# thourihan/DeepfakeDetection

Measured on AMD Instinct MI355X. Metric: train images/sec @224^2 (EfficientNet-B0), higher is better.
Workload: dtype bf16; 1 GPU; EfficientNet-b0 (timm flavour) 224x224 train step: bf16 fwd + label-smoothed CE + bwd + AdamW, random-init weights, 2 classes; per_gpu_batch=256, global_batch=256, parallelism=dp1, launch=hipgraph

## Files before the change

### deepfakedetection_amd/_lib.py

```python

from __future__ import annotations

import ctypes
from ctypes import POINTER, Structure, c_double, c_float, c_int, c_int64, c_long, c_size_t, c_uint32, c_void_p
from pathlib import Path

import os as _os

LIB_PATH = Path(_os.environ.get("DFD_LIB_PATH") or Path(__file__).resolve().parent / "libdfd_hip.so")

DFD_OK = 0
ERRORS = {-1: "DFD_EINVAL", -2: "DFD_EUNSUPPORTED", -3: "DFD_ELAUNCH", -4: "DFD_EWORKSPACE"}
F32, BF16 = 0, 1
ACT_NONE, ACT_SILU, ACT_RELU, ACT_GELU = 0, 1, 2, 3
PRO_NONE, PRO_BN_ACT, PRO_BN_ACT_GATE, PRO_AFFINE2 = 0, 1, 2, 3
MAX_PARTIALS = 1024
ADAMW_TABLE_COLS = 5
ADAMW_HP_LEN = 8
EMA_TABLE_COLS = 4
EMA_LERP, EMA_COPY = 0, 1
MIX_JOB_WORDS = 8
MIX_KEEP, MIX_MIXUP, MIX_CUTMIX = 0, 1, 2
MIX_NHWC, MIX_NCHW = 0, 1
AUG_MAX_OPS = 4
AUG_POLICY_JOB_WORDS = 16 + 2 + 9 * AUG_MAX_OPS


class DwShape(Structure):
    _fields_ = [(n, c_int) for n in ("N", "H", "W", "C", "Ho", "Wo", "k", "stride", "pad_top", "pad_left")]


class StemShape(Structure):
    _fields_ = [(n, c_int) for n in ("N", "H", "W", "Cout", "Ho", "Wo", "k", "stride", "pad_top", "pad_left")]


class Mat(Structure):

    _fields_ = [(n, c_long) for n in ("sb", "sh", "sr", "sc")]


class Prologue(Structure):
    _fields_ = [
        ("mode", c_int), ("act", c_int), ("HW", c_int), ("_pad", c_int),
        ("a2", c_void_p), ("coef", c_void_p), ("gate", c_void_p),
    ]


P = c_void_p
_PI = POINTER(c_int)

SIGNATURES: dict[str, tuple] = {
    "dfd_version": (c_int, []),
    "dfd_tune": (c_int, [c_int, c_int]),
    "dfd_dw_mm_plan": (c_int, [POINTER(DwShape), c_int, _PI]),
    "dfd_bn_finalize": (c_int, [P, c_int, c_int, c_double, P, P, P, P, c_float, c_float, P, P]),
    "dfd_bn_eval_coeffs": (c_int, [P, P, P, P, c_float, c_int, P, P]),
    "dfd_bn_bwd_finalize": (c_int, [P, c_int, c_int, c_double, P, P, c_int, P, P, c_int, P, P]),
    "dfd_bn_act_apply": (c_int, [c_int, P, P, c_int, P, P, P, c_int, c_int, c_int, P]),
    "dfd_bn_bwd_reduce": (c_int, [c_int, P, P, P, P, c_int, c_int, c_int, P, c_int, _PI, P]),
    "dfd_gemm_bias_act": (c_int, [c_int, P, P, c_int, c_int, c_int, P, c_int, P, P, c_int, P, P, P]),
    "dfd_gemm_plan": (c_int, [c_int, c_int, c_int]),
    "dfd_pw_ntd_plan": (c_int, [c_int, c_int, c_int]),
    "dfd_bias_grad_ws": (c_size_t, [c_int, c_int, c_int]),
    "dfd_bias_grad": (c_int, [c_int, P, P, c_int, c_int, c_int, P, c_int, P, c_size_t, P]),
    "dfd_act_bn_bwd": (c_int, [c_int, P, P, P, P, P, c_int, P, c_int, c_int, c_int, P, c_int, _PI, P]),
    "dfd_act_bn_bwd_se": (c_int, [c_int, P, P, P, P, P, c_int, P, c_int, c_int, c_int, P, c_int, _PI, P, P, c_int, P, P, P, P, c_int, P]),
    "dfd_prep_weights_multi": (c_int, [P, c_int, P]),
    "dfd_resize_crop_u8": (c_int, [P, P, P, c_int, c_int, c_int, c_int, P]),
    "dfd_augment_u8": (c_int, [P, P, P, c_int, c_int, c_int, P]),
    "dfd_image_prep": (c_int, [P, P, c_int, c_int, c_int, POINTER(c_float), POINTER(c_float), P, P, P]),
    "dfd_pool_ws": (c_size_t, [c_int, c_int, c_int, c_int]),
    "dfd_pool_act": (c_int, [c_int, P, P, c_int, P, c_int, c_int, c_int, P, c_size_t, P]),
    "dfd_pool_bwd_reduce": (c_int, [c_int, P, P, P, c_int, P, c_int, c_int, c_int, P, c_size_t, P]),
    "dfd_scale_rows": (c_int, [c_int, P, P, P, c_int, c_int, c_int, P]),
    "dfd_se_fc_fwd": (c_int, [P, P, P, P, P, c_int, c_int, c_int, c_int, P, P, P, P]),
    "dfd_se_fc_bwd": (c_int, [P, P, P, P, P, P, c_int, c_int, c_int, c_int, P, P, P, P, P, c_int, P, P]),
    "dfd_dwconv_fwd": (c_int, [c_int, P, P, c_int, P, P, POINTER(DwShape), P, c_int, _PI, P]),
    "dfd_dwconv_bwd_data": (c_int, [c_int, P, P, P, P, P, P, c_int, P, POINTER(DwShape), P, c_int, _PI, P]),
    "dfd_dwconv_bwd_weight": (c_int, [c_int, P, P, P, P, P, c_int, P, POINTER(DwShape), c_int, P, c_size_t, P]),
    "dfd_dwconv_bwd_weight_ws": (c_size_t, [POINTER(DwShape)]),
    "dfd_dwconv_bwd_fused": (c_int, [c_int, P, P, P, P, P, P, c_int, P, P, POINTER(DwShape), P, c_int, _PI, c_int, P, c_size_t, P]),
    "dfd_pwconv_fwd": (c_int, [c_int, P, POINTER(Prologue), P, P, P, c_int, c_int, c_int, P, c_int, _PI, P]),
    "dfd_pwconv_wgrad": (c_int, [c_int, P, POINTER(Prologue), c_int, P, POINTER(Prologue), c_int, c_int, P, c_int, P, c_size_t, P]),
    "dfd_pwconv_wgrad_ws": (c_size_t, [c_int, c_int, c_int]),
    "dfd_gradcam_map": (c_int, [P, P, c_int, c_int, c_int, c_int, P, P]),
    "dfd_cam_render": (c_int, [P, c_int, c_int, c_int, c_int, c_int, P, P, P, c_double, P, P, P, c_size_t, P]),
    "dfd_cam_render_ws": (c_size_t, [c_int, c_int, c_int, c_int, c_int]),
    "dfd_pwconv_bwd_fused": (c_int, [c_int, P, P, P, P, P, P, c_int, c_int, c_int, P, P, c_int, P, c_size_t, P]),
    "dfd_pw_prep_weights": (c_int, [c_int, P, P, P, c_int, c_int, P]),
    "dfd_stem_conv_fwd": (c_int, [c_int, P, P, P, POINTER(StemShape), P, c_int, _PI, P]),
    "dfd_stem_conv_wgrad": (c_int, [c_int, P, P, P, P, P, POINTER(StemShape), c_int, P, c_size_t, P]),
    "dfd_stem_conv_wgrad_ws": (c_size_t, [POINTER(StemShape)]),
    "dfd_dropout": (c_int, [P, P, c_float, P, c_int, P]),
    "dfd_linear_fwd": (c_int, [P, P, P, P, c_int, c_int, c_int, P]),
    "dfd_linear_bwd": (c_int, [P, P, P, P, P, P, c_int, c_int, c_int, c_int, P]),
    "dfd_ce_loss": (c_int, [P, P, c_int, c_int, c_float, c_float, P, P, P, P]),
    "dfd_softmax_argmax": (c_int, [P, c_int, c_int, P, P, P]),
    "dfd_adamw_step": (c_int, [P, c_int, P, P]),
    "dfd_ema_update": (c_int, [P, c_int, P, P]),
    "dfd_mix_batch": (c_int, [P, P, P, P, c_int, c_int, c_int, c_int, c_int, P]),
    "dfd_ce_loss_soft": (c_int, [P, P, c_int, c_int, c_float, c_float, P, P, P, P]),
    "dfd_augment_policy_u8": (c_int, [P, P, P, P, c_int, c_int, c_int, P]),
    "dfd_bn_eval_coeffs_multi": (c_int, [P, c_int, P]),
    "dfd_sum_batch_begin": (c_int, []),
    "dfd_sum_batch_end": (c_int, []),
    "dfd_sum_batch_end_deferred": (c_int, []),
    "dfd_sum_passengers_flush": (c_int, [P]),
    "dfd_sum_passengers_discard": (c_int, []),
    "dfd_se_fwd": (c_int, [c_int, P, P, c_int, c_int, c_int, c_int, P, P, P, P, c_int, c_int, P, P, P, P, P, c_size_t, P]),
    "dfd_se_bwd": (c_int, [c_int, P, P, P, c_int, c_int, c_int, c_int, P, P, P, P, P, c_int, c_int, P, P, P, P, P, P, c_int,
                           P, c_size_t, P, P]),
    "dfd_pwconv_fwd_eval": (c_int, [c_int, P, P, P, c_int, P, c_int, c_int, c_int, P]),
    "dfd_dwconv_fwd_eval_tiles": (c_int, [c_int, P]),
    "dfd_dwconv_fwd_eval": (c_int, [c_int, P, P, P, c_int, P, P, P, P, P]),
    "dfd_se_fwd_parts": (c_int, [P, c_int, c_int, c_int, c_int, P, P, P, P, c_int, c_int, P, P, P, P, P]),
    "dfd_bn_finalize_ex": (c_int, [P, c_int, c_int, c_double, P, P, P, P, P, P, c_float, c_float, P, P]),
    "dfd_bn_eval_coeffs_ex": (c_int, [P, P, P, P, P, P, c_float, c_int, P, P]),
    "dfd_bn_bwd_finalize_ex": (c_int, [P, c_int, c_int, c_double, P, P, P, P, c_int, P, P, P, P, c_int, P, P]),
    "dfd_affine2_apply": (c_int, [c_int, P, P, P, P, c_long, c_int, P]),
    "dfd_bn_add_act": (c_int, [c_int, P, P, P, c_int, P, c_long, c_int, P]),
    "dfd_bn_add_act_bwd": (c_int, [c_int, P, P, P, P, c_int, P, c_long, c_int, P, c_int, _PI, P]),
    "dfd_channel_stats": (c_int, [c_int, P, c_long, c_int, P, c_int, _PI, P]),
    "dfd_sum_rows": (c_int, [P, c_int, c_long, P, c_int, P]),
    "dfd_sum_rows_deferred": (c_int, [P, c_int, c_long, P, c_int, P]),
    "dfd_up2_act_fwd": (c_int, [c_int, P, c_int, P, c_int, c_int, c_int, c_int, P]),
    "dfd_up2_act_bwd": (c_int, [c_int, P, P, c_int, P, c_int, c_int, c_int, c_int, P, P]),
    "dfd_subsample_add": (c_int, [c_int, P, P, P, P, c_int, c_int, c_int, c_int, c_int, P]),
    "dfd_subsample_add_bwd": (c_int, [c_int, P, P, c_int, c_int, c_int, c_int, c_int, P]),
    "dfd_bgemm": (c_int, [c_int, P, POINTER(Mat), c_int, P, POINTER(Mat), c_int, P, POINTER(Mat), P, c_float, c_int, c_int,
                          c_int, c_int, c_int, c_int, c_int, P]),
    "dfd_attn_softmax_fwd": (c_int, [P, P, P, P, P, P, P, c_int, c_int, c_int, c_int, P]),
    "dfd_attn_softmax_bwd": (c_int, [P, P, P, P, P, P, c_int, c_int, c_int, c_int, P]),
    "dfd_bias_gather": (c_int, [P, P, P, c_int, c_int, c_long, P]),
    "dfd_bias_scatter": (c_int, [P, P, P, c_int, c_int, c_long, c_int, P]),
    "dfd_im2col": (c_int, [c_int, P, P, c_int, P, POINTER(DwShape), P]),
    "dfd_conv_fwd": (c_int, [c_int, P, POINTER(DwShape), P, c_int, P, c_int, P, P, c_int, POINTER(c_int), P]),
    "dfd_conv_wgrad_ws": (c_size_t, [POINTER(DwShape), c_int]),
    "dfd_conv_wgrad": (c_int, [c_int, P, P, c_int, P, POINTER(DwShape), P, c_int, P, c_int, P, c_size_t, P]),
    "dfd_col2im": (c_int, [c_int, P, P, POINTER(DwShape), P]),
    "dfd_conv_weight_perm": (c_int, [P, P, c_int, c_int, c_int, c_int, c_int, P]),
    "dfd_layernorm_fwd": (c_int, [c_int, P, P, P, c_float, P, P, c_long, c_int, P]),
    "dfd_layernorm_bwd": (c_int, [c_int, P, P, P, P, P, P, P, c_int, _PI, c_long, c_int, P]),
    "dfd_copy_rows": (c_int, [c_int, P, P, P, P, c_long, c_int, P]),
    "dfd_add_rowtable": (c_int, [c_int, P, P, P, c_long, c_int, c_int, P]),
    "dfd_rowtable_grad_ws": (c_size_t, [c_int, c_int]),
    "dfd_rowtable_grad": (c_int, [c_int, P, P, c_long, c_int, c_int, c_int, P, c_size_t, P]),
    "dfd_avgpool_fwd": (c_int, [c_int, P, P, c_int, c_int, c_int, c_int, c_int, c_int, P]),
    "dfd_avgpool_bwd": (c_int, [c_int, P, P, c_int, c_int, c_int, c_int, c_int, c_int, P]),
    "dfd_relpos_bias_fwd": (c_int, [P, P, P, c_int, c_int, c_int, P]),
    "dfd_relpos_bias_bwd": (c_int, [P, P, P, P, c_int, c_int, c_int, c_int, P]),
    "dfd_axpby": (c_int, [P, P, c_float, c_float, P, P, c_long, P]),
    "dfd_add": (c_int, [c_int, P, P, P, c_long, P]),
    "dfd_rand": (c_int, [P, c_uint32, c_float, P, c_long, P]),
    "dfd_step_tick": (c_int, [P, c_int, P, P]),
    "dfd_mx_quant_weights_multi": (c_int, [P, c_int, P]),
    "dfd_mx_quant_rows": (c_int, [c_int, P, POINTER(Prologue), P, P, c_long, c_int, P]),
    "dfd_mx_gemm": (c_int, [P, P, P, P, c_int, P, c_long, c_int, c_int, P]),
    "dfd_wattn_parts": (c_int, [c_int]),
    "dfd_wattn_fwd": (c_int, [P, P, P, P, c_int, c_int, c_int, c_int, c_float, P]),
    "dfd_wattn_bwd": (c_int, [P, P, P, P, P, P, c_int, c_int, c_int, c_int, c_float, P]),
    "dfd_attn_scores": (c_int, [P, P, P, P, c_float, c_int, c_int, c_int, c_int, c_int, P]),
    "dfd_attn_apply": (c_int, [P, c_int, P, P, c_float, c_int, c_int, c_int, c_int, c_int, P]),
    "dfd_coord_mlp_fwd_multi": (c_int, [P, c_int, P]),
    "dfd_coord_mlp_bwd_multi": (c_int, [P, c_int, P]),
    "dfd_relpos_bias_fwd_multi": (c_int, [P, c_int, P]),
    "dfd_relpos_bias_bwd_multi": (c_int, [P, c_int, P]),
}

class BnEvalJob(Structure):
    _fields_ = [("gamma", c_void_p), ("beta", c_void_p), ("conv_bias", c_void_p), ("ls", c_void_p), ("running_mean", c_void_p),
                ("running_var", c_void_p), ("bnstate", c_void_p), ("eps", c_float), ("C", c_int)]


class MxJob(Structure):

    _fields_ = [("src", c_void_p), ("q", c_void_p), ("scale", c_void_p), ("kn", c_void_p), ("N", c_int), ("K", c_int),
                ("kn_dtype", c_int), ("_pad", c_int)]


class CmlpJob(Structure):

    _fields_ = [(n, c_void_p) for n in ("coords", "w0", "b0", "w2", "table", "dtable", "dw0", "db0", "dw2")] + \
               [(n, c_int) for n in ("T", "D", "Hd", "_pad")]


class RelposJob(Structure):

    _fields_ = [(n, c_void_p) for n in ("table", "idx", "full", "dfull", "dtable")] + [(n, c_int) for n in ("H", "T", "n_local", "n_global")]


class PrepJob(Structure):

    _fields_ = [("src", c_void_p), ("nk", c_void_p), ("kn", c_void_p), ("N", c_int), ("K", c_int), ("dtype", c_int),
                ("_pad", c_int)]


_lib: ctypes.CDLL | None = None


def load() -> ctypes.CDLL:
    global _lib
    if _lib is not None:
        return _lib
    import torch

    if not LIB_PATH.exists():
        raise RuntimeError(
            f"{LIB_PATH} is missing: build it with `python -m deepfakedetection_amd.build` "
            "(hipcc --offload-arch=gfx950). There is no CPU fallback."
        )
    lib = ctypes.CDLL(str(LIB_PATH))
    for name, (restype, argtypes) in SIGNATURES.items():
        try:
            fn = getattr(lib, name)
        except AttributeError as exc:
            raise RuntimeError(f"libdfd_hip.so does not export {name}") from exc
        fn.restype = restype
        fn.argtypes = argtypes
    for item in filter(None, _os.environ.get("DFD_TUNE", "").split(",")):
        key, _, value = item.partition("=")
        if lib.dfd_tune(int(key), int(value)) != DFD_OK:
            raise RuntimeError(f"DFD_TUNE: unknown key in {item!r}")
    _lib = lib
    return lib


def check(code: int, op: str, detail: str = "") -> None:
    if code != DFD_OK:
        raise RuntimeError(f"{op} failed with {ERRORS.get(code, code)} {detail}")


__all__ = [
    "ACT_GELU", "ACT_NONE", "ACT_RELU", "ACT_SILU", "ADAMW_HP_LEN", "ADAMW_TABLE_COLS", "BF16", "EMA_COPY", "EMA_LERP", "EMA_TABLE_COLS", "F32",
    "MAX_PARTIALS", "MIX_CUTMIX", "MIX_JOB_WORDS", "MIX_KEEP", "MIX_MIXUP", "MIX_NCHW", "MIX_NHWC", "Mat", "PRO_AFFINE2", "PRO_BN_ACT", "PRO_BN_ACT_GATE", "PRO_NONE", "DwShape", "Prologue",
    "StemShape", "SIGNATURES", "check", "load", "c_int64",
]
```

### deepfakedetection_amd/csrc/dfd_misc.hip

```cpp
#include "dfd_common.h"
#include "dfd_se.h"

__device__ __forceinline__ float wave_sum(float v) {
#pragma unroll
    for (int o = 32; o >= 1; o >>= 1) v += __shfl_xor(v, o);
    return v;
}
__device__ __forceinline__ float wave_max(float v) {
#pragma unroll
    for (int o = 32; o >= 1; o >>= 1) v = fmaxf(v, __shfl_xor(v, o));
    return v;
}
template <int ACT> __device__ __forceinline__ float act_rt(float z) { return act_fwd<ACT>(z); }

#define SE_MAX_C 4096
#define SE_MAX_R 128

__device__ __forceinline__ float wave_dot(const float* __restrict__ a, const float* __restrict__ b, int C, int lane) {
    float s = 0.f;
    for (int c = lane * 4; c < C; c += 256) {
        const float4 x = *reinterpret_cast<const float4*>(a + c);
        const float4 y = *reinterpret_cast<const float4*>(b + c);
        s = fmaf(x.x, y.x, fmaf(x.y, y.y, fmaf(x.z, y.z, fmaf(x.w, y.w, s))));
    }
// ... 128 lines not shown
                const int r = rb + k * NW;
                if (r < R) {
                    const float z = s4[k] + (b1 ? b1[r] : 0.f);
                    hpre[(long)n * R + r] = z;
                    sh[r] = act_rt<ACT>(z);
                }
            }
        }
    }
    __syncthreads();
    for (int c = t; c < C; c += SE_IMG_THREADS) {
        float s = b2 ? b2[c] : 0.f;
        int r = 0;
        for (; r + 8 <= R; r += 8) {
            float wv[8];
#pragma unroll
            for (int u = 0; u < 8; ++u) wv[u] = w2t[(long)(r + u) * C + c];
#pragma unroll
            for (int u = 0; u < 8; ++u) s = fmaf(wv[u], sh[r + u], s);
        }
        for (; r < R; ++r) s = fmaf(w2t[(long)r * C + c], sh[r], s);
        gate[(long)n * C + c] = sigmoid_f(s);
    }
}

template <int ACT>
__global__ void __launch_bounds__(SE_IMG_THREADS)
k_se_bwd_img(const float* __restrict__ parts, int splits, const float* __restrict__ dgate_in, const float* __restrict__ gate,
             const float* __restrict__ hpre, const float* __restrict__ w1, const float* __restrict__ w2t, int N, int C, int R,
             float* __restrict__ ws, float* __restrict__ dpooled) {
    __shared__ __attribute__((aligned(16))) float sp[SE_MAX_C];
    __shared__ float sd[SE_MAX_R];
    float* ws_g = ws;
    float* ws_dh = ws + (long)N * C;
    float* ws_h = ws_dh + (long)N * R;
    constexpr int NW = SE_IMG_THREADS / 64;
    const int n = blockIdx.x, t = threadIdx.x, lane = t & 63, wave = t >> 6;
    for (int c = t; c < C; c += SE_IMG_THREADS) {
        float d;
        if (splits > 1) {
            d = 0.f;
            for (int z = 0; z < splits; ++z) d += parts[((long)z * N + n) * C + c];
        } else {
            d = dgate_in[(long)n * C + c];
        }
        const float g = gate[(long)n * C + c];
        const float v = d * g * (1.f - g);
        ws_g[(long)n * C + c] = v;
        sp[c] = v;
    }
    __syncthreads();
    for (int rb = wave; rb < R; rb += 4 * NW) {
        float s4[4];
        lds_dot4(sp, w2t, C, R, rb, NW, lane, s4);
        if (lane == 0) {
#pragma unroll
            for (int k = 0; k < 4; ++k) {
                const int r = rb + k * NW;
                if (r < R) {
                    const float z = hpre[(long)n * R + r];
                    const float dh = s4[k] * act_grad<ACT>(z);
                    ws_dh[(long)n * R + r] = dh;
                    ws_h[(long)n * R + r] = act_rt<ACT>(z);
                    sd[r] = dh;
                }
            }
        }
    }
    __syncthreads();
    for (int c = t; c < C; c += SE_IMG_THREADS) {
        float s = 0.f;
        int r = 0;
        for (; r + 8 <= R; r += 8) {
            float wv[8];
#pragma unroll
            for (int u = 0; u < 8; ++u) wv[u] = w1[(long)(r + u) * C + c];
#pragma unroll
            for (int u = 0; u < 8; ++u) s = fmaf(sd[r + u], wv[u], s);
        }
        for (; r < R; ++r) s = fmaf(sd[r], w1[(long)r * C + c], s);
        dpooled[(long)n * C + c] = s;
    }
}

__global__ void k_transpose_f32(const float* __restrict__ in, float* __restrict__ out, int rows, int cols) {
    const int i = blockIdx.x * blockDim.x + threadIdx.x;
    if (i >= rows * cols) return;
    const int c = i / rows, r = i - c * rows;
    out[i] = in[(long)r * cols + c];
}

extern "C" int dfd_se_fc_fwd(const float* pooled, const float* w1, const float* b1, const float* w2, const float* b2,
                             int N, int C, int R, int act, float* hpre, float* gate, float* w2t, dfd_stream stream) {
    if (!pooled || !w1 || !hpre || !gate || !w2t || N < 1 || C < 1 || R < 1) return DFD_EINVAL;
    if (C > SE_MAX_C || R > SE_MAX_R) return DFD_EUNSUPPORTED;
    hipStream_t st = (hipStream_t)stream;
    if (w2) hipLaunchKernelGGL(k_transpose_f32, dim3((C * R + 255) / 256), dim3(256), 0, st, w2, w2t, C, R);
    hipLaunchKernelGGL(k_se_hidden, dim3((R + 3) / 4, N), dim3(DFD_THREADS), 0, st, pooled, w1, b1, C, R, hpre);
    DISPATCH_ACT(act, {
        hipLaunchKernelGGL((k_se_gate<ACT>), dim3((C + DFD_THREADS - 1) / DFD_THREADS, N), dim3(DFD_THREADS), 0, st, hpre, w2t,
                           b2, C, R, gate);
    });
    return DFD_CHECK_LAUNCH();
}

extern "C" int dfd_se_fwd(int dtype, const void* y, const float* bnstate, int act_in, int N, int HW, int C, const float* w1,
                          const float* b1, const float* w2, const float* b2, int R, int act, float* pooled, float* hpre,
                          float* gate, float* w2t, void* ws, size_t ws_bytes, dfd_stream stream) {
    if (!y || !bnstate || !w1 || !pooled || !hpre || !gate || !w2t || N < 1 || C < 1 || R < 1 || C % 4) return DFD_EINVAL;
    if (C > SE_MAX_C || R > SE_MAX_R) return DFD_EUNSUPPORTED;
    hipStream_t st = (hipStream_t)stream;
    if (w2) hipLaunchKernelGGL(k_transpose_f32, dim3((C * R + 255) / 256), dim3(256), 0, st, w2, w2t, C, R);
    int splits = 1;
    float mul = 1.f;
    const int rc = dfd_pool_launch(dtype, false, nullptr, y, bnstate, act_in, pooled, N, HW, C, ws, ws_bytes, st, &splits, &mul);
    if (rc != DFD_OK) return rc;
    DISPATCH_ACT(act, {
        hipLaunchKernelGGL((k_se_fwd_img<ACT>), dim3(N), dim3(SE_IMG_THREADS), 0, st, splits > 1 ? (const float*)ws : nullptr, splits,
                           mul, pooled, w1, b1, w2t, b2, N, C, R, hpre, gate);
    });
    return DFD_CHECK_LAUNCH();
}

extern "C" int dfd_se_fwd_parts(const float* parts, int splits, int N, int HW, int C, const float* w1, const float* b1,
                                const float* w2, const float* b2, int R, int act, float* pooled, float* hpre, float* gate,
                                float* w2t, dfd_stream stream) {
    if (!parts || splits < 1 || !w1 || !pooled || !hpre || !gate || !w2t || N < 1 || HW < 1 || C < 1 || R < 1 || C % 4) return DFD_EINVAL;
    if (C > SE_MAX_C || R > SE_MAX_R) return DFD_EUNSUPPORTED;
    hipStream_t st = (hipStream_t)stream;
    if (w2) hipLaunchKernelGGL(k_transpose_f32, dim3((C * R + 255) / 256), dim3(256), 0, st, w2, w2t, C, R);
    DISPATCH_ACT(act, {
        hipLaunchKernelGGL((k_se_fwd_img<ACT>), dim3(N), dim3(SE_IMG_THREADS), 0, st, parts, splits, 1.f / (float)HW, pooled, w1, b1,
                           w2t, b2, N, C, R, hpre, gate);
    });
    return DFD_CHECK_LAUNCH();
}

extern "C" int dfd_se_bwd(int dtype, const void* D, const void* y, const float* bnstate, int act_in, int N, int HW, int C,
                          const float* gate, const float* hpre, const float* pooled, const float* w1, const float* w2t, int R,
                          int act, float* dgate, float* dpooled, float* dw1, float* db1, float* dw2, float* db2, int accumulate,
                          void* pool_ws, size_t pool_ws_bytes, float* ws, dfd_stream stream) {
    if (!D || !y || !bnstate || !gate || !hpre || !pooled || !w1 || !w2t || !dgate || !dpooled || !ws || N < 1 || C < 1 ||
        R < 1 || C % 4)
        return DFD_EINVAL;
    if (C > SE_MAX_C || R > SE_MAX_R) return DFD_EUNSUPPORTED;
    hipStream_t st = (hipStream_t)stream;
    int splits = 1;
    float mul = 1.f;
    const int rc = dfd_pool_launch(dtype, true, D, y, bnstate, act_in, dgate, N, HW, C, pool_ws, pool_ws_bytes, st, &splits, &mul);
    if (rc != DFD_OK) return rc;
    DISPATCH_ACT(act, {
        hipLaunchKernelGGL((k_se_bwd_img<ACT>), dim3(N), dim3(SE_IMG_THREADS), 0, st, (const float*)pool_ws, splits, dgate, gate, hpre,
                           w1, w2t, N, C, R, ws, dpooled);
    });
    if (hipGetLastError() != hipSuccess) return DFD_ELAUNCH;
    if (dw1 && dw2) {
        hipLaunchKernelGGL(k_se_fc_bwd_w, dim3((C + 63) / 64, R), dim3(DFD_THREADS), 0, st, pooled, ws, N, C, R, dw1, db1,
                           dw2, db2, accumulate);
    }
    return DFD_CHECK_LAUNCH();
}

extern "C" int dfd_se_fc_bwd(const float* dgate, const float* gate, const float* hpre, const float* pooled,
                             const float* w1, const float* w2t, int N, int C, int R, int act, float* dpooled,
                             float* dw1, float* db1, float* dw2, float* db2, int accumulate, float* ws,
                             dfd_stream stream) {
    if (!dgate || !gate || !hpre || !pooled || !w1 || !w2t || !dpooled || !ws || N < 1 || C < 1 || R < 1) return DFD_EINVAL;
    if (C > SE_MAX_C || R > SE_MAX_R) return DFD_EUNSUPPORTED;
    hipStream_t st = (hipStream_t)stream;
    DISPATCH_ACT(act, {
        hipLaunchKernelGGL((k_se_bwd_hidden<ACT>), dim3((R + 3) / 4, N), dim3(DFD_THREADS), 0, st, dgate, gate, hpre, w2t, N, C,
                           R, ws);
    });
    hipLaunchKernelGGL(k_se_bwd_pooled, dim3((C + DFD_THREADS - 1) / DFD_THREADS, N), dim3(DFD_THREADS), 0, st, ws, w1, N, C, R,
                       dpooled);
    if (hipGetLastError() != hipSuccess) return DFD_ELAUNCH;
    if (dw1 && dw2) {
        hipLaunchKernelGGL(k_se_fc_bwd_w, dim3((C + 63) / 64, R), dim3(DFD_THREADS), 0, st, pooled, ws, N, C, R, dw1, db1,
                           dw2, db2, accumulate);
    }
    return DFD_CHECK_LAUNCH();
}

#define STEM_MAX_CO 64
template <typename T, int K>
__global__ void __launch_bounds__(DFD_THREADS)
k_stem_fwd(const float* __restrict__ x, const float* __restrict__ w, T* __restrict__ y, dfd_stem_shape s, ChanMap cm,
           float* __restrict__ partials, int stats) {
    constexpr int V = Vec<T>::N;
    constexpr int TAPS = 3 * K * K;
    __shared__ __attribute__((aligned(16))) float wl[TAPS * STEM_MAX_CO];
    __shared__ float red[DFD_THREADS * 2 * V];
    const int t = threadIdx.x, vl = t % cm.cvb, rl = t / cm.cvb;
    const bool active = rl < cm.rpb;
    const int Co = s.Cout, c0 = vl * V;
    for (int i = t; i < TAPS * Co; i += DFD_THREADS) {
        const int tap = i / Co, co = i - tap * Co;
        wl[tap * Co + co] = round_to<T>(w[(long)co * TAPS + tap]);
    }
    __syncthreads();
    float s1[V], s2[V];
#pragma unroll
    for (int j = 0; j < V; ++j) { s1[j] = 0.f; s2[j] = 0.f; }
    const long npix = (long)s.N * s.Ho * s.Wo;
    if (active) {
        const long step = (long)gridDim.x * cm.rpb;
        for (long pix = (long)blockIdx.x * cm.rpb + rl; pix < npix; pix += step) {
            const int ox = (int)(pix % s.Wo);
            const long tq = pix / s.Wo;
            const int oy = (int)(tq % s.Ho);
            const long n = tq / s.Ho;
            typedef float f2v __attribute__((ext_vector_type(2)));
            f2v acc2[V / 2];
#pragma unroll
            for (int j = 0; j < V / 2; ++j) acc2[j] = (f2v){0.f, 0.f};
            const int ix0 = ox * s.stride - s.pad_left;
            const bool row_inside = ix0 >= 0 && ix0 + K <= s.W && K == 3;
#pragma unroll
            for (int kh = 0; kh < K; ++kh) {
                const int iy = oy * s.stride - s.pad_top + kh;
                if (iy < 0 || iy >= s.H) continue;
                float xr[3 * K];
                const float* prow = x + ((n * s.H + iy) * (long)s.W + ix0) * 3;
                if (row_inside) {
                    struct __attribute__((packed, aligned(4))) F4 { float a, b, c, d; };
                    const F4 q0 = *reinterpret_cast<const F4*>(prow), q1 = *reinterpret_cast<const F4*>(prow + 4);
                    xr[0] = q0.a; xr[1] = q0.b; xr[2] = q0.c; xr[3] = q0.d;
                    xr[4] = q1.a; xr[5] = q1.b; xr[6] = q1.c; xr[7] = q1.d;
                    xr[8] = prow[8];
                } else {
#pragma unroll
                    for (int kw = 0; kw < K; ++kw) {
                        const int ix = ix0 + kw;
                        const bool ok = ix >= 0 && ix < s.W;
#pragma unroll
                        for (int ci = 0; ci < 3; ++ci) xr[kw * 3 + ci] = ok ? prow[kw * 3 + ci] : 0.f;
                    }
                }
#pragma unroll
                for (int kw = 0; kw < K; ++kw)
#pragma unroll
                    for (int ci = 0; ci < 3; ++ci) {
                        const float xv = round_to<T>(xr[kw * 3 + ci]);
                        const f2v xx = (f2v){xv, xv};
                        const float* wp = wl + ((ci * K + kh) * K + kw) * Co + c0;
                        f2v wv[V / 2];
#pragma unroll
                        for (int j4 = 0; j4 < V / 4; ++j4) {
                            const float4 q = *reinterpret_cast<const float4*>(wp + 4 * j4);
                            wv[2 * j4] = (f2v){q.x, q.y};
                            wv[2 * j4 + 1] = (f2v){q.z, q.w};
                        }
#pragma unroll
                        for (int j = 0; j < V / 2; ++j) acc2[j] = __builtin_elementwise_fma(xx, wv[j], acc2[j]);
                    }
            }
            float acc[V];
#pragma unroll
            for (int j = 0; j < V / 2; ++j) { acc[2 * j] = acc2[j].x; acc[2 * j + 1] = acc2[j].y; }
#pragma unroll
            for (int j = 0; j < V; ++j) {
                const float r = round_to<T>(acc[j]);
                acc[j] = r;
                s1[j] += r;
                s2[j] = fmaf(r, r, s2[j]);
            }
            Vec<T>::store(y + pix * Co + c0, acc);
        }
    }
    if (stats) {
        float acc2[2 * V];
#pragma unroll
        for (int j = 0; j < V; ++j) { acc2[j] = s1[j]; acc2[V + j] = s2[j]; }
        reduce_rowlanes<2 * V>(acc2, red, cm.cvb, cm.rpb, vl, rl, active);
        if (rl == 0) {
            float* p = partials + (long)blockIdx.x * 2 * Co;
            float a0[V], a1[V];
#pragma unroll
            for (int j = 0; j < V; ++j) { a0[j] = acc2[j]; a1[j] = acc2[V + j]; }
            store_f32<V>(p + c0, a0);
            store_f32<V>(p + Co + c0, a1);
        }
    }
}

#define STEM_CHUNK 128
#define STEM_TAPP 32
template <typename T, int K>
__global__ void __launch_bounds__(DFD_THREADS)
k_stem_wgrad(const float* __restrict__ x, const T* __restrict__ dz, const T* __restrict__ yraw,
             const float* __restrict__ coef, dfd_stem_shape s, float* __restrict__ ws) {
    constexpr int V = Vec<T>::N;
    constexpr int TAPS = 3 * K * K;
    static_assert(TAPS <= STEM_TAPP, "patch padding");
    __shared__ __attribute__((aligned(16))) float sdy[STEM_CHUNK * STEM_MAX_CO];
    __shared__ __attribute__((aligned(16))) float sx[STEM_CHUNK * STEM_TAPP];
    const int t = threadIdx.x, Co = s.Cout;
    const int COG = Co / 4, TPG = COG * 4, NG = DFD_THREADS / TPG;
    const int grp = t / TPG, r = t - grp * TPG, cog = r >> 2, tg = r & 3;
    const bool on = grp < NG;
    float acc[4][8];
#pragma unroll
    for (int i = 0; i < 4; ++i)
#pragma unroll
        for (int j = 0; j < 8; ++j) acc[i][j] = 0.f;
    for (int i = t; i < STEM_CHUNK * STEM_TAPP; i += DFD_THREADS) sx[i] = 0.f;
// ... 532 lines not shown
```

### deepfakedetection_amd/csrc/dfd_pwtnw.hip

```cpp
#include "dfd_pw.h"

#define TNW_MIN_ROWS 16

template <int ROWS, int NA, int NBT, int PA, int PB, int ACT, int DG = 0>
__global__ void __launch_bounds__(DFD_THREADS, NBT > 9 ? 1 : 2)
k_pw_tnw(const bf16* __restrict__ a, ProArgs pa, int Na, const bf16* __restrict__ b, ProArgs pb, int Nb, int M,
         int rows_per_block, int swap, float* __restrict__ ws, const bf16* __restrict__ w_kn = nullptr,
         const bf16* __restrict__ res = nullptr, bf16* __restrict__ dx = nullptr, int wstride = 0, int woff = 0) {
    constexpr int ITA = (ROWS * NA * 2 + 63) / 64;
    constexpr int ITB = (ROWS * NBT * 2 + 63) / 64;
    extern __shared__ __attribute__((aligned(16))) unsigned char smem[];
    const int t = threadIdx.x, lane = t & 63, wave = t >> 6;
    unsigned char* at = smem + wave * (2 * ROWS * 256);
    unsigned char* bt = at + ROWS * 256;
    float* cl = reinterpret_cast<float*>(smem + 4 * 2 * ROWS * 256);
    const bf16* a2 = reinterpret_cast<const bf16*>(pa.a2);
    const bf16* b2 = reinterpret_cast<const bf16*>(pb.a2);
    const int ca = Na >> 3, cb = Nb >> 3;
    float* gc = cl + 3 * (Na + Nb) + wave * 2 * Nb;
    int gimg = -1;

    for (int i = t; i < 3 * Na; i += DFD_THREADS) cl[i] = (PA != DFD_PRO_NONE) ? pa.coef[i] : 0.f;
    for (int i = t; i < 3 * Nb; i += DFD_THREADS) {
        float v = 0.f;
        if (PB == DFD_PRO_AFFINE2) v = pb.coef[i];
        else if (PB != DFD_PRO_NONE && i < 2 * Nb) v = pb.coef[i];
        cl[3 * Na + i] = v;
    }
    for (int i = t; i < 4 * 2 * ROWS * 256 / 16; i += DFD_THREADS) reinterpret_cast<uint4*>(smem)[i] = make_uint4(0, 0, 0, 0);
    if constexpr (DG) {
        const int chunks = wstride >> 4;
        for (int i = t; i < NA * 16 * chunks; i += DFD_THREADS) {
            const int r = i / chunks, c = i - r * chunks;
            uint4 v = make_uint4(0, 0, 0, 0);
            if (r < Na && c < cb) v = *reinterpret_cast<const uint4*>(w_kn + (long)r * Nb + c * 8);
            *reinterpret_cast<uint4*>(smem + woff + r * wstride + c * 16) = v;
        }
    }
    __syncthreads();

    int ra[ITA], cha[ITA], rb[ITB], chb[ITB];
#pragma unroll
    for (int i = 0; i < ITA; ++i) {
        const int idx = lane + 64 * i;
        const bool ok = idx < ROWS * ca;
        ra[i] = ok ? idx / ca : -1;
        cha[i] = ok ? idx - ra[i] * ca : 0;
    }
#pragma unroll
    for (int i = 0; i < ITB; ++i) {
        const int idx = lane + 64 * i;
        const bool ok = idx < ROWS * cb;
        rb[i] = ok ? idx / cb : -1;
        chb[i] = ok ? idx - rb[i] * cb : 0;
    }

    f32x4_t acc[NA][NBT];
#pragma unroll
    for (int x = 0; x < NA; ++x)
#pragma unroll
        for (int y = 0; y < NBT; ++y) acc[x][y] = (f32x4_t){0.f, 0.f, 0.f, 0.f};
    const int na = (Na + 15) >> 4, nbt = (Nb + 15) >> 4;
    constexpr int RT = ROWS / 16;
    f32x4_t accd[DG ? NA : 1][RT];

    const int rows_per_wave = rows_per_block / 4;
    const int mbeg = blockIdx.x * rows_per_block + wave * rows_per_wave;
    int mend = mbeg + rows_per_wave;
    if (mend > M) mend = M;

    uint4 va[ITA], va2[ITA], vb[ITB], vb2[ITB];
    auto load_a = [&](int i, int m0) {
        int row = m0 + (ra[i] < 0 ? 0 : ra[i]);
        row = row < M ? row : M - 1;
        const long off = (long)row * Na + cha[i] * 8;
        va[i] = *reinterpret_cast<const uint4*>(a + off);
        if constexpr (PA == DFD_PRO_AFFINE2) va2[i] = *reinterpret_cast<const uint4*>(a2 + off);
    };
    auto load_b = [&](int i, int m0) {
        int row = m0 + (rb[i] < 0 ? 0 : rb[i]);
        row = row < M ? row : M - 1;
        const long off = (long)row * Nb + chb[i] * 8;
        vb[i] = *reinterpret_cast<const uint4*>(b + off);
        if constexpr (PB == DFD_PRO_AFFINE2) vb2[i] = *reinterpret_cast<const uint4*>(b2 + off);
    };
    auto g_load = [&](int m0) {
#pragma unroll
        for (int i = 0; i < ITA; ++i) load_a(i, m0);
#pragma unroll
        for (int i = 0; i < ITB; ++i) load_b(i, m0);
    };
    auto pro_item = [&](auto mode_tag, uint4 q, uint4 q2, const float* cf, int N, int ch, int m, const ProArgs& pr) -> uint4 {
        constexpr int MODE = decltype(mode_tag)::value;
        if constexpr (MODE == DFD_PRO_NONE) {
            return q;
        } else {
            float v[8], c0[8], c1[8];
            q_to_f(q, v);
            load_f32<8>(cf + ch * 8, c0);
            load_f32<8>(cf + N + ch * 8, c1);
            if constexpr (MODE == DFD_PRO_AFFINE2) {
                float v2[8], c2[8];
                q_to_f(q2, v2);
                load_f32<8>(cf + 2 * N + ch * 8, c2);
#pragma unroll
                for (int j = 0; j < 8; ++j) v[j] = fmaf(c0[j], v[j], fmaf(c1[j], v2[j], c2[j]));
            } else if constexpr (MODE == DFD_PRO_BN_ACT) {
                bn_act_array<ACT, 8>(v, c0, c1);
            } else {
                float gt[8];
                load_f32<8>(gc + (pro_image(pr, m) - gimg) * N + ch * 8, gt);
                bn_act_array<ACT, 8>(v, c0, c1);
#pragma unroll
                for (int j = 0; j < 8; ++j) v[j] = round_to<bf16>(v[j]) * gt[j];
            }
            return f_to_q(v);
        }
    };
    auto s_store_a = [&](int m0) {
#pragma unroll
        for (int i = 0; i < ITA; ++i) {
            if (ra[i] >= 0) {
                uint4 v = make_uint4(0, 0, 0, 0);
                if (m0 + ra[i] < mend) v = pro_item(std::integral_constant<int, PA>{}, va[i], va2[i], cl, Na, cha[i], m0 + ra[i], pa);
                *reinterpret_cast<uint4*>(at + tn_off_bf16(ra[i], cha[i])) = v;
            }
            load_a(i, m0 + ROWS);
        }
    };
    auto s_store_b = [&](int m0, int grp, auto refill_tag) {
        constexpr bool refill = decltype(refill_tag)::value;
#pragma unroll
        for (int i = 0; i < ITB; ++i) {
            if (rb[i] >= 0 && (chb[i] >> 4) == grp) {
                uint4 v = make_uint4(0, 0, 0, 0);
                if (m0 + rb[i] < mend)
                    v = pro_item(std::integral_constant<int, PB>{}, vb[i], vb2[i], cl + 3 * Na, Nb, chb[i], m0 + rb[i], pb);
                *reinterpret_cast<uint4*>(bt + tn_off_bf16(rb[i], chb[i] & 15)) = v;
            }
            if constexpr (refill) load_b(i, m0 + ROWS);
        }
    };
    auto wave_sync = [&]() {
        __builtin_amdgcn_fence(__ATOMIC_RELEASE, "wavefront");
        __builtin_amdgcn_wave_barrier();
        __builtin_amdgcn_fence(__ATOMIC_ACQUIRE, "wavefront");
    };
    const int g = lane >> 4, li = lane & 15, qrow = li >> 2, pcol = li & 3;
    auto frag = [&](const unsigned char* tile, int ch0) -> short8_t {
        const int ch = ch0 + (pcol >> 1), sub = (pcol & 1) << 3;
        if constexpr (ROWS == 32) {
            const int m_lo = 8 * g + qrow, m_hi = m_lo + 4;
            const short4_t lo = __builtin_amdgcn_ds_read_tr16_b64_v4i16(
                (__attribute__((address_space(3))) short4_t*)(tile + tn_off_bf16(m_lo, ch) + sub));
            const short4_t hi = __builtin_amdgcn_ds_read_tr16_b64_v4i16(
                (__attribute__((address_space(3))) short4_t*)(tile + tn_off_bf16(m_hi, ch) + sub));
            return (short8_t){lo[0], lo[1], lo[2], lo[3], hi[0], hi[1], hi[2], hi[3]};
        } else {
            const short4_t lo = __builtin_amdgcn_ds_read_tr16_b64_v4i16(
                (__attribute__((address_space(3))) short4_t*)(tile + tn_off_bf16(4 * g + qrow, ch) + sub));
            return (short8_t){lo[0], lo[1], lo[2], lo[3], 0, 0, 0, 0};
        }
    };
    auto mma = [&](const short8_t& fx, const short8_t& fy, f32x4_t c) -> f32x4_t {
        if constexpr (ROWS == 32) {
            return __builtin_amdgcn_mfma_f32_16x16x32_bf16(__builtin_bit_cast(bf16x8_t, fx), __builtin_bit_cast(bf16x8_t, fy), c, 0, 0, 0);
        } else {
            const short4_t x4 = (short4_t){fx[0], fx[1], fx[2], fx[3]}, y4 = (short4_t){fy[0], fy[1], fy[2], fy[3]};
            return __builtin_amdgcn_mfma_f32_16x16x16bf16_1k(x4, y4, c, 0, 0, 0);
        }
    };

    constexpr int NGRP = NBT > 8 ? 2 : 1;
    if (mbeg < mend) g_load(mbeg);
    for (int m0 = mbeg; m0 < mend; m0 += ROWS) {
        short8_t fa[NA];
        if constexpr (PB == DFD_PRO_BN_ACT_GATE) {
            const int img0 = pro_image(pb, m0);
            if (img0 != gimg) {
                gimg = img0;
                for (int i = lane; i < 2 * Nb; i += 64) {
                    const int im = img0 + (i >= Nb ? 1 : 0);
                    gc[i] = ((long)im * pb.HW < M) ? pb.gate[(long)im * Nb + (i >= Nb ? i - Nb : i)] : 0.f;
                }
                wave_sync();
            }
        }
        if constexpr (DG) {
#pragma unroll
            for (int x = 0; x < NA; ++x)
#pragma unroll
                for (int j = 0; j < RT; ++j) accd[x][j] = (f32x4_t){0.f, 0.f, 0.f, 0.f};
        }
        s_store_a(m0);
        s_store_b(m0, 0, std::integral_constant<bool, NGRP == 1>{});
        wave_sync();
#pragma unroll
        for (int x = 0; x < NA; ++x)
            if (x < na) fa[x] = frag(at, 2 * x);
#pragma unroll
        for (int grp = 0; grp < NGRP; ++grp) {
            if (grp > 0) {
                wave_sync();
                s_store_b(m0, grp, std::true_type{});
                wave_sync();
            }
#pragma unroll
            for (int y = 0; y < NBT; ++y) {
                if ((y >> 3) != grp || y >= nbt) continue;
                const short8_t fb = frag(bt, 2 * (y & 7));
#pragma unroll
                for (int x = 0; x < NA; ++x)
                    if (x < na)
                        acc[x][y] = mma(fa[x], fb, acc[x][y]);
            }
            if constexpr (DG) {
#pragma unroll
                for (int ks = 0; ks < 4; ++ks) {
                    if (grp * 8 + 2 * ks >= NBT || grp * 8 + 2 * ks >= nbt) continue;
                    const int chl = 4 * ks + g, chg = grp * 16 + chl;
                    uint4 fd[RT];
#pragma unroll
                    for (int j = 0; j < RT; ++j) {
                        fd[j] = *reinterpret_cast<const uint4*>(bt + tn_off_bf16(j * 16 + li, chl));
                        if (chg >= cb) fd[j] = make_uint4(0, 0, 0, 0);
                    }
#pragma unroll
                    for (int x = 0; x < NA; ++x) {
                        if (x >= na) continue;
                        const uint4 fw = *reinterpret_cast<const uint4*>(smem + woff + (x * 16 + li) * wstride + chg * 16);
#pragma unroll
                        for (int j = 0; j < RT; ++j)
                            accd[x][j] = __builtin_amdgcn_mfma_f32_16x16x32_bf16(__builtin_bit_cast(bf16x8_t, fw), __builtin_bit_cast(bf16x8_t, fd[j]),
                                                                               accd[x][j], 0, 0, 0);
                    }
                }
            }
        }
        if constexpr (DG) {
#pragma unroll
            for (int j = 0; j < RT; ++j) {
                const int m = m0 + j * 16 + li;
#pragma unroll
                for (int x = 0; x < NA; ++x) {
                    const int ci = x * 16 + 4 * g;
                    if (x < na && m < mend && ci < Na) {
                        float v[4];
#pragma unroll
                        for (int r = 0; r < 4; ++r) v[r] = round_to<bf16>(accd[x][j][r]);
                        if constexpr (DG == 2) {
                            const uint2 rq = *reinterpret_cast<const uint2*>(res + (long)m * Na + ci);
                            v[0] = round_to<bf16>(v[0] + __uint_as_float(rq.x << 16)); v[1] = round_to<bf16>(v[1] + __uint_as_float(rq.x & 0xffff0000u));
                            v[2] = round_to<bf16>(v[2] + __uint_as_float(rq.y << 16)); v[3] = round_to<bf16>(v[3] + __uint_as_float(rq.y & 0xffff0000u));
                        }
                        *reinterpret_cast<uint2*>(dx + (long)m * Na + ci) = make_uint2(pack_bf2(v[0], v[1]), pack_bf2(v[2], v[3]));
                    }
                }
            }
        }
        wave_sync();
    }

    __syncthreads();
    float* red = reinterpret_cast<float*>(smem);
    for (int w = 0; w < 4; ++w) {
        if (wave == w) {
#pragma unroll
            for (int x = 0; x < NA; ++x)
#pragma unroll
                for (int y = 0; y < NBT; ++y) {
                    if (x >= na || y >= nbt) continue;
                    float* r = red + ((x * NBT + y) * 64 + lane) * 4;
                    float4 cur = w == 0 ? make_float4(0.f, 0.f, 0.f, 0.f) : *reinterpret_cast<float4*>(r);
                    cur.x += acc[x][y][0]; cur.y += acc[x][y][1]; cur.z += acc[x][y][2]; cur.w += acc[x][y][3];
                    *reinterpret_cast<float4*>(r) = cur;
                }
        }
        __syncthreads();
    }
    float* o = ws + (long)blockIdx.x * Na * Nb;
    for (int e = t; e < na * nbt * 256; e += DFD_THREADS) {
        const int tile = e >> 8, l = (e >> 2) & 63, r = e & 3;
        const int x = tile / nbt, y = tile - x * nbt;
        const int ia = x * 16 + (l >> 4) * 4 + r, jb = y * 16 + (l & 15);
        if (ia < Na && jb < Nb) {
            const float v = red[((x * NBT + y) * 64 + l) * 4 + r];
            if (swap) o[(long)jb * Na + ia] = v; else o[(long)ia * Nb + jb] = v;
        }
    }
}

static bool tnw_pro_ok(int mode_narrow, int mode_wide) {
    return (mode_narrow == DFD_PRO_NONE || mode_narrow == DFD_PRO_AFFINE2) &&
           (mode_wide == DFD_PRO_NONE || mode_wide == DFD_PRO_AFFINE2 || mode_wide == DFD_PRO_BN_ACT_GATE ||
            mode_wide == DFD_PRO_BN_ACT);
}

template <int ROWS, int NA, int NBT>
static int tnw_launch(const void* a, const dfd_prologue* pro_a, int Na, const void* b, const dfd_prologue* pro_b, int Nb,
                      int M, int swap, float* dw, int accumulate, float* ws, size_t ws_bytes, hipStream_t st) {
    const ProArgs pa = pro_args(pro_a), pb = pro_args(pro_b);
    const int ma = pro_a ? pro_a->mode : DFD_PRO_NONE, mb = pro_b ? pro_b->mode : DFD_PRO_NONE;
    const int act = ((mb == DFD_PRO_BN_ACT_GATE || mb == DFD_PRO_BN_ACT) && pro_b) ? pro_b->act : DFD_ACT_NONE;
    int nblocks = 512;
    int rpb = (M + nblocks - 1) / nblocks;
    rpb = (rpb + 4 * ROWS - 1) / (4 * ROWS) * (4 * ROWS);
    nblocks = (M + rpb - 1) / rpb;
    if ((size_t)(nblocks + nblocks / 32 + 2) * Na * Nb * 4 > ws_bytes) return DFD_EUNSUPPORTED;
    const bool gated = mb == DFD_PRO_BN_ACT_GATE;
    if (gated && pb.HW < ROWS) return DFD_EUNSUPPORTED;
    const int lds = 4 * 2 * ROWS * 256 + 3 * (Na + Nb) * 4 + (gated ? 4 * 2 * Nb * 4 : 0);
#define LAUNCH_TNW(PAV, PBV, ACTV)                                                                                     \
    hipLaunchKernelGGL((k_pw_tnw<ROWS, NA, NBT, PAV, PBV, ACTV>), dim3(nblocks), dim3(DFD_THREADS), lds, st, (const bf16*)a, pa, \
                       Na, (const bf16*)b, pb, Nb, M, rpb, swap, ws)
    if (mb == DFD_PRO_BN_ACT_GATE) {
        if (act != DFD_ACT_SILU) return DFD_EUNSUPPORTED;
        if (ma == DFD_PRO_AFFINE2) LAUNCH_TNW(DFD_PRO_AFFINE2, DFD_PRO_BN_ACT_GATE, DFD_ACT_SILU);
        else LAUNCH_TNW(DFD_PRO_NONE, DFD_PRO_BN_ACT_GATE, DFD_ACT_SILU);
    } else if (mb == DFD_PRO_BN_ACT) {
        if (ma != DFD_PRO_AFFINE2) return DFD_EUNSUPPORTED;
        if (act == DFD_ACT_GELU) LAUNCH_TNW(DFD_PRO_AFFINE2, DFD_PRO_BN_ACT, DFD_ACT_GELU);
        else if (act == DFD_ACT_SILU) LAUNCH_TNW(DFD_PRO_AFFINE2, DFD_PRO_BN_ACT, DFD_ACT_SILU);
        else return DFD_EUNSUPPORTED;
    } else if (mb == DFD_PRO_AFFINE2) {
        if (ma == DFD_PRO_AFFINE2) return DFD_EUNSUPPORTED;
        LAUNCH_TNW(DFD_PRO_NONE, DFD_PRO_AFFINE2, DFD_ACT_NONE);
    } else {
        if (ma == DFD_PRO_AFFINE2) LAUNCH_TNW(DFD_PRO_AFFINE2, DFD_PRO_NONE, DFD_ACT_NONE);
        else LAUNCH_TNW(DFD_PRO_NONE, DFD_PRO_NONE, DFD_ACT_NONE);
    }
#undef LAUNCH_TNW
    if (hipGetLastError() != hipSuccess) return DFD_ELAUNCH;
    return dfd_launch_sum_partials(ws, nblocks, (long)Na * Nb, dw, accumulate, st);
}

template <int ROWS, int NA, int NBT>
static int tnw_dg_launch(const void* x, int Cin, const void* dz, const dfd_prologue* pro_d, int Cm, const void* w_kn, const void* residual,
                         int M, void* dx, float* dw, int accumulate, float* ws, size_t ws_bytes, hipStream_t st) {
    const ProArgs pa = pro_args(nullptr), pb = pro_args(pro_d);
    int nblocks = NBT > 9 ? 256 : 512;
    int rpb = (M + nblocks - 1) / nblocks;
    rpb = (rpb + 4 * ROWS - 1) / (4 * ROWS) * (4 * ROWS);
    nblocks = (M + rpb - 1) / rpb;
    if ((size_t)(nblocks + nblocks / 32 + 2) * Cin * Cm * 4 > ws_bytes) return DFD_EUNSUPPORTED;
    const int wstride = (Cm + 31) / 32 * 64 + 16;
    int woff = 4 * 2 * ROWS * 256 + 3 * (Cin + Cm) * 4;
    woff = (woff + 15) / 16 * 16;
    const int lds = woff + NA * 16 * wstride;
    if (lds > 80 * 1024) return DFD_EUNSUPPORTED;
    struct TnwDgTag;
    dfd_allow_lds_once<TnwDgTag>(k_pw_tnw<ROWS, NA, NBT, DFD_PRO_NONE, DFD_PRO_AFFINE2, DFD_ACT_NONE, 2>, 80 * 1024);
    dfd_allow_lds_once<TnwDgTag>(k_pw_tnw<ROWS, NA, NBT, DFD_PRO_NONE, DFD_PRO_AFFINE2, DFD_ACT_NONE, 1>, 80 * 1024);
    if (residual)
        hipLaunchKernelGGL((k_pw_tnw<ROWS, NA, NBT, DFD_PRO_NONE, DFD_PRO_AFFINE2, DFD_ACT_NONE, 2>), dim3(nblocks), dim3(DFD_THREADS), lds, st,
                           (const bf16*)x, pa, Cin, (const bf16*)dz, pb, Cm, M, rpb, 1, ws, (const bf16*)w_kn, (const bf16*)residual, (bf16*)dx,
                           wstride, woff);
    else
        hipLaunchKernelGGL((k_pw_tnw<ROWS, NA, NBT, DFD_PRO_NONE, DFD_PRO_AFFINE2, DFD_ACT_NONE, 1>), dim3(nblocks), dim3(DFD_THREADS), lds, st,
                           (const bf16*)x, pa, Cin, (const bf16*)dz, pb, Cm, M, rpb, 1, ws, (const bf16*)w_kn, (const bf16*)nullptr, (bf16*)dx,
                           wstride, woff);
    if (hipGetLastError() != hipSuccess) return DFD_ELAUNCH;
    return dfd_launch_sum_partials(ws, nblocks, (long)Cin * Cm, dw, accumulate, st);
}
extern "C" int dfd_pwconv_bwd_fused(int dtype, const void* dz, const void* y, const float* coef, const void* x, const void* w_kn,
                                    const void* residual, int M, int Cm, int Cin, void* dx, float* dw, int accumulate, float* ws,
                                    size_t ws_bytes, dfd_stream stream) {
    if (!dz || !y || !coef || !x || !w_kn || !dx || !dw || !ws || M < 1 || Cm < 8 || Cin < 8 || Cm % 8 || Cin % 8) return DFD_EINVAL;
    if (dtype != DFD_BF16 || M < 2048 * 32 * 3 || Cin > 48 || Cin > Cm || !(Cm <= 128 || (Cm <= 240 && Cm % 16 == 0))) return DFD_EUNSUPPORTED;
    if (Cin > 32 && Cm <= 144) return DFD_EUNSUPPORTED;
    dfd_prologue pro{};
    pro.mode = DFD_PRO_AFFINE2; pro.act = DFD_ACT_NONE; pro.HW = 1; pro.a2 = y; pro.coef = coef; pro.gate = nullptr;
    hipStream_t st = (hipStream_t)stream;
    if (Cm <= 96) return tnw_dg_launch<32, 2, 6>(x, Cin, dz, &pro, Cm, w_kn, residual, M, dx, dw, accumulate, ws, ws_bytes, st);
    if (Cm <= 144) return tnw_dg_launch<16, 2, 9>(x, Cin, dz, &pro, Cm, w_kn, residual, M, dx, dw, accumulate, ws, ws_bytes, st);
    if (Cm <= 192) return tnw_dg_launch<16, 3, 12>(x, Cin, dz, &pro, Cm, w_kn, residual, M, dx, dw, accumulate, ws, ws_bytes, st);
    return tnw_dg_launch<16, 3, 15>(x, Cin, dz, &pro, Cm, w_kn, residual, M, dx, dw, accumulate, ws, ws_bytes, st);
}

int dfd_pw_tnw(const void* p, const dfd_prologue* pro_p, int Ni, const void* q, const dfd_prologue* pro_q, int Nj, int M,
               float* dw, int accumulate, float* ws, size_t ws_bytes, hipStream_t st) {
    if (M < 2048 * 32 * 3) return DFD_EUNSUPPORTED;
    const int mp = pro_p ? pro_p->mode : DFD_PRO_NONE, mq = pro_q ? pro_q->mode : DFD_PRO_NONE;
    const auto wide_ok = [](int n) { return n <= 128 || (n <= 144 && n % 16 == 0); };
#define TNW_PICK(NARROW, WIDE, ...)                                             \
    do {                                                                       \
        if ((NARROW) <= 32 && (WIDE) <= 96) return tnw_launch<32, 2, 6>(__VA_ARGS__); \
        if ((NARROW) <= 32) return tnw_launch<16, 2, 9>(__VA_ARGS__);               \
        return DFD_EUNSUPPORTED;     \
    } while (0)
    if (Ni <= 48 && wide_ok(Nj) && Ni <= Nj && tnw_pro_ok(mp, mq))
        TNW_PICK(Ni, Nj, p, pro_p, Ni, q, pro_q, Nj, M, 0, dw, accumulate, ws, ws_bytes, st);
    if (Nj <= 48 && wide_ok(Ni) && tnw_pro_ok(mq, mp))
        TNW_PICK(Nj, Ni, q, pro_q, Nj, p, pro_p, Ni, M, 1, dw, accumulate, ws, ws_bytes, st);
#undef TNW_PICK
    return DFD_EUNSUPPORTED;
}
```

### deepfakedetection_amd/csrc/dfd_rowpass.hip

```cpp
#include "dfd_common.h"
#include "dfd_se.h"
#include "dfd_sum.h"

template <typename T, int ACT, bool HAS_RES, bool HAS_RS>
__global__ void __launch_bounds__(DFD_THREADS)
k_bn_act_apply(const T* __restrict__ y, const float* __restrict__ bnstate, const T* __restrict__ res,
               const float* __restrict__ rs, T* __restrict__ out, long total_vec, int CV, int C, long vec_per_img) {
    constexpr int V = Vec<T>::N;
    const long stride = (long)gridDim.x * DFD_THREADS;
    const long first = (long)blockIdx.x * DFD_THREADS + threadIdx.x;
    int cv = (int)(first % CV);
    const int cstep = (int)(stride % CV);
    for (long i = first; i < total_vec; i += stride, cv = cv + cstep >= CV ? cv + cstep - CV : cv + cstep) {
        const int c0 = cv * V;
        float v[V], sc[V], sh[V];
        Vec<T>::load(y + i * V, v);
        load_f32<V>(bnstate + c0, sc);
        load_f32<V>(bnstate + C + c0, sh);
        float r = 1.f;
        if constexpr (HAS_RS) r = rs[i / vec_per_img];
        float q[V];
        if constexpr (HAS_RES) Vec<T>::load(res + i * V, q);
        bn_act_array<ACT, V>(v, sc, sh);
#pragma unroll
// ... 529 lines not shown
    s = (HW + rp - 1) / rp;
    *splits = s;
    *rows_per = rp;
}
static size_t pool_ws_bytes(int N, int HW, int C, int vec) {
    int s, rp;
    pool_plan(N, HW, C, vec, &s, &rp);
    if (s <= 1) return 0;
    return (size_t)s * N * C * sizeof(float);
}
extern "C" int dfd_act_bn_bwd_se(int dtype, const void* D, const void* y, const float* gate, const float* dpool,
                                 const float* bnstate, int act, void* dz, int N, int HW, int C, float* partials, int pcap,
                                 int* nparts, const float* se_pooled, const float* se_ws, int R, float* dw1, float* db1, float* dw2,
                                 float* db2, int accumulate, dfd_stream stream) {
    if (!shape_ok(dtype, N, HW, C) || !y || !bnstate || !dz || !partials || !nparts || pcap < 1) return DFD_EINVAL;
    if (!se_pooled || !se_ws || !dw1 || !dw2 || R < 1) return DFD_EINVAL;
    const SeWgradJob job{se_pooled, se_ws, N, C, R, dw1, db1, dw2, db2, accumulate};
    hipStream_t st = (hipStream_t)stream;
    return dtype == DFD_BF16
               ? act_bn_bwd_t<bf16>(D, y, gate, dpool, bnstate, act, dz, N, HW, C, partials, pcap, nparts, st, &job)
               : act_bn_bwd_t<float>(D, y, gate, dpool, bnstate, act, dz, N, HW, C, partials, pcap, nparts, st, &job);
}

extern "C" size_t dfd_pool_ws(int dtype, int N, int HW, int C) {
    if (!shape_ok(dtype, N, HW, C)) return 0;
    return pool_ws_bytes(N, HW, C, dtype == DFD_BF16 ? Vec<bf16>::N : Vec<float>::N);
}

template <typename T, bool BWD>
static int pool_t(const void* D, const void* y, const float* bnstate, int act, float* out, int N, int HW, int C,
                  void* ws, size_t ws_bytes, hipStream_t st, int* defer = nullptr, float* mul_out = nullptr) {
    const ChanMap cm = make_chanmap(C, Vec<T>::N);
    int splits = 1, rows_per = HW;
    if (ws) {
        pool_plan(N, HW, C, Vec<T>::N, &splits, &rows_per);
        if (splits > 1 && pool_ws_bytes(N, HW, C, Vec<T>::N) > ws_bytes) return DFD_EWORKSPACE;
    }
    float* parts = splits > 1 ? (float*)ws : nullptr;
    dim3 grid(cm.nvc, N, splits);
    const float mul = BWD ? 1.0f : 1.0f / (float)HW;
    DISPATCH_ACT(act, {
        hipLaunchKernelGGL((k_pool<T, ACT, BWD>), grid, dim3(DFD_THREADS), 0, st, (const T*)D, (const T*)y, bnstate, out, HW,
                           C, mul, cm, rows_per, parts);
    });
    if (defer) {
        *defer = splits;
        *mul_out = mul;
    } else if (splits > 1) {
        const long NC = (long)N * C;
        hipLaunchKernelGGL(k_pool_sum, dim3((unsigned)((NC + 255) / 256)), dim3(256), 0, st, parts, splits, NC, mul, out);
    }
    return DFD_CHECK_LAUNCH();
}
int dfd_pool_launch(int dtype, bool bwd, const void* D, const void* y, const float* bnstate, int act, float* out, int N,
                    int HW, int C, void* ws, size_t ws_bytes, hipStream_t st, int* splits, float* mul) {
    if (!shape_ok(dtype, N, HW, C) || !y || !bnstate || !out || (bwd && !D)) return DFD_EINVAL;
    if (dtype == DFD_BF16)
        return bwd ? pool_t<bf16, true>(D, y, bnstate, act, out, N, HW, C, ws, ws_bytes, st, splits, mul)
                   : pool_t<bf16, false>(nullptr, y, bnstate, act, out, N, HW, C, ws, ws_bytes, st, splits, mul);
    return bwd ? pool_t<float, true>(D, y, bnstate, act, out, N, HW, C, ws, ws_bytes, st, splits, mul)
               : pool_t<float, false>(nullptr, y, bnstate, act, out, N, HW, C, ws, ws_bytes, st, splits, mul);
}
extern "C" int dfd_pool_act(int dtype, const void* y, const float* bnstate, int act, float* pooled, int N, int HW,
                            int C, void* ws, size_t ws_bytes, dfd_stream stream) {
    if (!shape_ok(dtype, N, HW, C) || !y || !bnstate || !pooled) return DFD_EINVAL;
    hipStream_t st = (hipStream_t)stream;
    return dtype == DFD_BF16 ? pool_t<bf16, false>(nullptr, y, bnstate, act, pooled, N, HW, C, ws, ws_bytes, st)
                             : pool_t<float, false>(nullptr, y, bnstate, act, pooled, N, HW, C, ws, ws_bytes, st);
}
extern "C" int dfd_pool_bwd_reduce(int dtype, const void* D, const void* y, const float* bnstate, int act,
                                   float* dgate, int N, int HW, int C, void* ws, size_t ws_bytes, dfd_stream stream) {
    if (!shape_ok(dtype, N, HW, C) || !D || !y || !bnstate || !dgate) return DFD_EINVAL;
    hipStream_t st = (hipStream_t)stream;
    return dtype == DFD_BF16 ? pool_t<bf16, true>(D, y, bnstate, act, dgate, N, HW, C, ws, ws_bytes, st)
                             : pool_t<float, true>(D, y, bnstate, act, dgate, N, HW, C, ws, ws_bytes, st);
}

extern "C" int dfd_bn_finalize_ex(const float* partials, int nparts, int C, double count, const float* gamma,
                                  const float* beta, const float* conv_bias, const float* ls_gamma, float* running_mean,
                                  float* running_var, float momentum, float eps, float* bnstate, dfd_stream stream) {
    if (!partials || nparts < 1 || C < 1 || count <= 0 || !bnstate) return DFD_EINVAL;
    if ((running_mean == nullptr) != (running_var == nullptr)) return DFD_EINVAL;
    const int threads = FIN_CH * FIN_LANES, grid = (C + FIN_CH - 1) / FIN_CH;
    hipLaunchKernelGGL(k_bn_finalize, dim3(grid), dim3(threads), 0, (hipStream_t)stream, partials, nparts, C, count, gamma,
                       beta, conv_bias, ls_gamma, running_mean, running_var, momentum, eps, bnstate);
    return DFD_CHECK_LAUNCH();
}
extern "C" int dfd_bn_finalize(const float* partials, int nparts, int C, double count, const float* gamma,
                               const float* beta, float* running_mean, float* running_var, float momentum, float eps,
                               float* bnstate, dfd_stream stream) {
    return dfd_bn_finalize_ex(partials, nparts, C, count, gamma, beta, nullptr, nullptr, running_mean, running_var, momentum,
                              eps, bnstate, stream);
}
extern "C" int dfd_bn_eval_coeffs_ex(const float* gamma, const float* beta, const float* conv_bias, const float* ls_gamma,
                                     const float* running_mean, const float* running_var, float eps, int C, float* bnstate,
                                     dfd_stream stream) {
    if (!running_mean || !running_var || C < 1 || !bnstate) return DFD_EINVAL;
    const int threads = 256, grid = (C + threads - 1) / threads;
    hipLaunchKernelGGL(k_bn_eval_coeffs, dim3(grid), dim3(threads), 0, (hipStream_t)stream, gamma, beta, conv_bias, ls_gamma,
                       running_mean, running_var, eps, C, bnstate);
    return DFD_CHECK_LAUNCH();
}
#define BN_EVAL_JOBS_PER_LAUNCH 40
struct BnEvalJobs { dfd_bn_eval_job j[BN_EVAL_JOBS_PER_LAUNCH]; };
__global__ void k_bn_eval_coeffs_multi(BnEvalJobs J) {
    const dfd_bn_eval_job& b = J.j[blockIdx.y];
    const int c = blockIdx.x * blockDim.x + threadIdx.x;
    if (c >= b.C) return;
    const float rstd = 1.0f / sqrtf(b.running_var[c] + b.eps);
    const float g = b.gamma ? b.gamma[c] : 1.f, be = b.beta ? b.beta[c] : 0.f;
    const float m = b.running_mean[c] - (b.conv_bias ? b.conv_bias[c] : 0.f);
    const float l = b.ls ? b.ls[c] : 1.f;
    const float scale = g * rstd;
    b.bnstate[c] = l * scale;
    b.bnstate[b.C + c] = l * (be - m * scale);
    b.bnstate[2 * b.C + c] = m;
    b.bnstate[3 * b.C + c] = rstd;
}
extern "C" int dfd_bn_eval_coeffs_multi(const dfd_bn_eval_job* jobs, int njobs, dfd_stream stream) {
    if (!jobs || njobs < 1) return DFD_EINVAL;
    for (int i = 0; i < njobs; ++i)
        if (!jobs[i].running_mean || !jobs[i].running_var || !jobs[i].bnstate || jobs[i].C < 1) return DFD_EINVAL;
    for (int base = 0; base < njobs; base += BN_EVAL_JOBS_PER_LAUNCH) {
        BnEvalJobs J;
        const int cnt = njobs - base < BN_EVAL_JOBS_PER_LAUNCH ? njobs - base : BN_EVAL_JOBS_PER_LAUNCH;
        int maxC = 0;
        for (int i = 0; i < cnt; ++i) { J.j[i] = jobs[base + i]; if (J.j[i].C > maxC) maxC = J.j[i].C; }
        hipLaunchKernelGGL(k_bn_eval_coeffs_multi, dim3((maxC + 255) / 256, cnt), dim3(256), 0, (hipStream_t)stream, J);
    }
    return DFD_CHECK_LAUNCH();
}
extern "C" int dfd_bn_eval_coeffs(const float* gamma, const float* beta, const float* running_mean,
                                  const float* running_var, float eps, int C, float* bnstate, dfd_stream stream) {
    return dfd_bn_eval_coeffs_ex(gamma, beta, nullptr, nullptr, running_mean, running_var, eps, C, bnstate, stream);
}
extern "C" int dfd_bn_bwd_finalize_ex(const float* partials, int nparts, int C, double count, const float* gamma,
                                      const float* beta, const float* ls_gamma, const float* bnstate, int train,
                                      float* dgamma, float* dbeta, float* dls, float* dbias, int accumulate, float* coef,
                                      dfd_stream stream) {
    if (!partials || nparts < 1 || C < 1 || count <= 0 || !bnstate || !coef) return DFD_EINVAL;
    if (dls && (!ls_gamma || !beta)) return DFD_EINVAL;
    const int threads = FIN_CH * FIN_LANES, grid = (C + FIN_CH - 1) / FIN_CH;
    hipLaunchKernelGGL(k_bn_bwd_finalize, dim3(grid), dim3(threads), 0, (hipStream_t)stream, partials, nparts, C, count,
                       gamma, beta, ls_gamma, bnstate, train, dgamma, dbeta, dls, dbias, accumulate, coef);
    return DFD_CHECK_LAUNCH();
}
extern "C" int dfd_bn_bwd_finalize(const float* partials, int nparts, int C, double count, const float* gamma,
                                   const float* bnstate, int train, float* dgamma, float* dbeta, int accumulate,
                                   float* coef, dfd_stream stream) {
    return dfd_bn_bwd_finalize_ex(partials, nparts, C, count, gamma, nullptr, nullptr, bnstate, train, dgamma, dbeta, nullptr,
                                  nullptr, accumulate, coef, stream);
}

extern "C" int dfd_version(void) { return 139; }
```

### deepfakedetection_amd/functions.py

```python

from __future__ import annotations

import contextlib
import os
import threading
from dataclasses import dataclass

import torch

from . import kernels as K
from ._lib import ACT_NONE, ACT_SILU
from .arch import ConvGeom
from .arena import grad_dest


@dataclass
class BNRef:

    running_mean: torch.Tensor
    running_var: torch.Tensor
    num_batches_tracked: torch.Tensor | None
    momentum: float
    eps: float
    pre: torch.Tensor | None = None
# ... 57 lines not shown

def _ptrs(*tensors) -> tuple[int, ...]:
    return tuple(t.data_ptr() if isinstance(t, torch.Tensor) else 0 for t in tensors)


def _dest(ctx, index: int, shape):
    if not ctx.needs_input_grad[index] or not ctx.pptr[index]:
        return None
    return grad_dest(ctx.pptr[index], shape)


@dataclass
class StemCtx:
    geom: ConvGeom
    bn: BNRef
    dtype: torch.dtype
    training: bool
    counters: list | None = None


class StemFunction(torch.autograd.Function):

    @staticmethod
    def forward(ctx, x, weight, gamma, beta, cfg: StemCtx):
        g = cfg.geom
        N, H, W, _ = x.shape
        Ho, Wo = g.out_size(H), g.out_size(W)
        y, parts, n = K.stem_conv_fwd(x, weight, cfg.dtype, g.stride, g.pad_lead, g.pad_lead, Ho, Wo, stats=cfg.training)
        st = _bn_state(parts, n, N * Ho * Wo, cfg.bn, gamma, beta, cfg.training, cfg.counters)
        out = K.bn_act_apply(y, st, ACT_SILU)
        ctx.cfg = cfg
        ctx.pptr = _ptrs(x, weight, gamma, beta)
        ctx.save_for_backward(x, y, st, gamma)
        return out

    @staticmethod
    def backward(ctx, g):
        cfg: StemCtx = ctx.cfg
        x, y, st, gamma = ctx.saved_tensors
        geom = cfg.geom
        N, Ho, Wo, _ = y.shape
        dz, parts, n = K.act_bn_bwd(_c(g), y, None, None, st, ACT_SILU)
        want_bn = ctx.needs_input_grad[2] or ctx.needs_input_grad[3]
        C = gamma.numel()
        coef, dgamma, dbeta = K.bn_bwd_finalize(parts, n, N * Ho * Wo, gamma, st, cfg.training, want_bn,
                                                _dest(ctx, 2, (C,)), _dest(ctx, 3, (C,)))
        dw = None
        if ctx.needs_input_grad[1]:
            dw = K.stem_conv_wgrad(x, dz, y, coef, geom.kernel, geom.stride, geom.pad_lead, geom.pad_lead,
                                   _dest(ctx, 1, (C, 3, geom.kernel, geom.kernel)))
        return None, dw, dgamma, dbeta, None


@dataclass
class MBConvCtx:
    expand: bool
    dw: ConvGeom
    skip: bool
    bn_expand: BNRef | None
    bn_dw: BNRef
    bn_project: BNRef
    training: bool
    derived: tuple | None = None
    counters: list | None = None
    grad_enabled: bool = True


class MBConvFunction(torch.autograd.Function):

    @staticmethod
    def forward(ctx, x, w_exp, g_exp, b_exp, w_dw, g_dw, b_dw, se_w1, se_b1, se_w2, se_b2, w_proj, g_proj, b_proj,
                row_scale, cfg: MBConvCtx):
        tr = cfg.training
        N, H, W, Cin = x.shape
        dt = x.dtype
        geom = cfg.dw
        Ho, Wo = geom.out_size(H), geom.out_size(W)
        need_bwd = any(ctx.needs_input_grad)
        if not tr and not (need_bwd and cfg.grad_enabled) and eval_fused_enabled(
                N * H * W * (w_exp.shape[0] if cfg.expand else Cin), dt):
            return MBConvFunction._forward_eval(x, w_exp, g_exp, b_exp, w_dw, g_dw, b_dw, se_w1, se_b1, se_w2, se_b2, w_proj,
                                                g_proj, b_proj, cfg, Ho, Wo)
        if cfg.expand:
            wexp_nk, wexp_kn = cfg.derived[0] if cfg.derived is not None else K.prep_weights(w_exp, dt, True, need_bwd)
            y1, parts, n = K.pwconv(x, None, wexp_nk, None, stats=tr)
            st1 = _bn_state(parts, n, N * H * W, cfg.bn_expand, g_exp, b_exp, tr, cfg.counters)
            y2, parts, n = K.dwconv_fwd(y1, st1, ACT_SILU, w_dw, geom.kernel, geom.stride, geom.pad_lead, geom.pad_lead,
                                        Ho, Wo, stats=tr)
        else:
            wexp_kn, y1, st1 = None, None, None
            y2, parts, n = K.dwconv_fwd(x, None, ACT_NONE, w_dw, geom.kernel, geom.stride, geom.pad_lead, geom.pad_lead,
                                        Ho, Wo, stats=tr)
        st2 = _bn_state(parts, n, N * Ho * Wo, cfg.bn_dw, g_dw, b_dw, tr, cfg.counters)
        w1, w2 = se_w1.reshape(se_w1.shape[0], -1), se_w2.reshape(se_w2.shape[0], -1)
        pooled, hpre, gate, w2t = K.se_fwd(y2, st2, ACT_SILU, w1, se_b1, w2, se_b2, ACT_SILU,
                                           cfg.derived[2] if cfg.derived is not None else None)
        wproj_nk, wproj_kn = cfg.derived[1] if cfg.derived is not None else K.prep_weights(w_proj, dt, True, need_bwd)
        pro = K.pro_bn_act_gate(st2, ACT_SILU, gate, Ho * Wo)
        y3, parts, n = K.pwconv(y2, pro, wproj_nk, None, stats=tr)
        st3 = _bn_state(parts, n, N * Ho * Wo, cfg.bn_project, g_proj, b_proj, tr, cfg.counters)
        out = K.bn_act_apply(y3, st3, ACT_NONE, x if cfg.skip else None, row_scale if cfg.skip else None)
        ctx.cfg = cfg
        ctx.pptr = _ptrs(x, w_exp, g_exp, b_exp, w_dw, g_dw, b_dw, se_w1, se_b1, se_w2, se_b2, w_proj, g_proj, b_proj)
        ctx.in_shape = (N, H, W, Cin)
        ctx.has_rs = cfg.skip and row_scale is not None
        ctx.save_for_backward(x, y1, y2, y3, st1, st2, st3, pooled, hpre, gate, wexp_kn, wproj_kn, w_dw, w1, w2t,
                              g_exp, g_dw, g_proj, row_scale if ctx.has_rs else None)
        return out

    @staticmethod
    def _forward_eval(x, w_exp, g_exp, b_exp, w_dw, g_dw, b_dw, se_w1, se_b1, se_w2, se_b2, w_proj, g_proj, b_proj, cfg, Ho, Wo):
        N, H, W, Cin = x.shape
        dt = x.dtype
        geom = cfg.dw
        a1 = x
        if cfg.expand:
            wexp_nk, _ = cfg.derived[0] if cfg.derived is not None else K.prep_weights(w_exp, dt, True, False)
            st1 = _bn_state(None, 0, N * H * W, cfg.bn_expand, g_exp, b_exp, False, cfg.counters)
            a1 = K.pwconv_eval(x, wexp_nk, st1, ACT_SILU)
        st2 = _bn_state(None, 0, N * Ho * Wo, cfg.bn_dw, g_dw, b_dw, False, cfg.counters)
        a2, pool_parts, _ = K.dwconv_eval(a1, w_dw, st2, ACT_SILU, geom.kernel, geom.stride, geom.pad_lead, geom.pad_lead, Ho, Wo)
        w1, w2 = se_w1.reshape(se_w1.shape[0], -1), se_w2.reshape(se_w2.shape[0], -1)
        _, gate, _ = K.se_fwd_parts(pool_parts, Ho * Wo, w1, se_b1, w2, se_b2, ACT_SILU,
                                    cfg.derived[2] if cfg.derived is not None else None)
        wproj_nk, _ = cfg.derived[1] if cfg.derived is not None else K.prep_weights(w_proj, dt, True, False)
        pro = K.pro_bn_act_gate(K.identity_state(x.device, a2.shape[3]), ACT_NONE, gate, Ho * Wo)
        y3, _, _ = K.pwconv(a2, pro, wproj_nk, None, stats=False)
        st3 = _bn_state(None, 0, N * Ho * Wo, cfg.bn_project, g_proj, b_proj, False, cfg.counters)
        return K.bn_act_apply(y3, st3, ACT_NONE, x if cfg.skip else None, None)

    @staticmethod
    def backward(ctx, g):
        cfg: MBConvCtx = ctx.cfg
        (x, y1, y2, y3, st1, st2, st3, pooled, hpre, gate, wexp_kn, wproj_kn, w_dw, w1, w2t,
         g_exp, g_dw, g_proj, row_scale) = ctx.saved_tensors
        need = ctx.needs_input_grad
        tr = cfg.training
        geom = cfg.dw
        N, H, W, Cin = ctx.in_shape
        _, Ho, Wo, Cmid = y2.shape
        with K.sum_batch():
            return MBConvFunction._backward(ctx, g, cfg, x, y1, y2, y3, st1, st2, st3, pooled, hpre, gate, wexp_kn, wproj_kn,
                                            w_dw, w1, w2t, g_exp, g_dw, g_proj, row_scale, need, tr, geom, N, H, W, Cin, Ho, Wo, Cmid)

    @staticmethod
    def _backward(ctx, g, cfg, x, y1, y2, y3, st1, st2, st3, pooled, hpre, gate, wexp_kn, wproj_kn, w_dw, w1, w2t, g_exp, g_dw,
                  g_proj, row_scale, need, tr, geom, N, H, W, Cin, Ho, Wo, Cmid):
        g = _c(g)
        gb = K.scale_rows(g, row_scale) if ctx.has_rs else g
        parts, n = K.bn_bwd_reduce(gb, y3, st3, None)
        Cout, R = y3.shape[3], w1.shape[0]
        coef3, dg_proj, db_proj = K.bn_bwd_finalize(parts, n, N * Ho * Wo, g_proj, st3, tr, need[12] or need[13],
                                                    _dest(ctx, 12, (Cout,)), _dest(ctx, 13, (Cout,)))
        gm3 = K.affine2_apply(gb, y3, coef3)
        D, _, _ = K.pwconv(gm3, None, wproj_kn, None, stats=False)
        dw_proj = None
        if need[11]:
            pro_q = K.pro_bn_act_gate(st2, ACT_SILU, gate, Ho * Wo)
            with K.side_stream(N * Ho * Wo):
                dw_proj = K.pwconv_wgrad(gm3, None, y2, pro_q, _dest(ctx, 11, (Cout, Cmid))).view(Cout, Cmid, 1, 1)
        want_se = need[7] or need[8] or need[9] or need[10]
        se_outs = (_dest(ctx, 7, (R, Cmid)), _dest(ctx, 8, (R,)), _dest(ctx, 9, (Cmid, R)), _dest(ctx, 10, (Cmid,)))
        se_res = K.se_bwd(D, y2, st2, ACT_SILU, gate, hpre, pooled, w1, w2t, ACT_SILU, want_se, se_outs, defer_wgrad=SE_WGRAD_PASSENGER)
        dpooled, dw1, db1, dw2, db2 = se_res[:5]
        se_job = se_res[5] if SE_WGRAD_PASSENGER else None
        dz2, parts, n = K.act_bn_bwd(D, y2, gate, dpooled, st2, ACT_SILU, se_job=se_job)
        if dw1 is not None:
            dw1, dw2 = dw1.view(dw1.shape[0], -1, 1, 1), dw2.view(dw2.shape[0], -1, 1, 1)
        coef2, dg_dw, db_dw = K.bn_bwd_finalize(parts, n, N * Ho * Wo, g_dw, st2, tr, need[5] or need[6],
                                                _dest(ctx, 5, (Cmid,)), _dest(ctx, 6, (Cmid,)))
        kk = geom.kernel
        dw_dw = dx = dw_exp = dg_exp = db_exp = None
        if cfg.expand:
            fused = need[4] and K.dwconv_bwd_fused_ok(geom.kernel, geom.stride)
            if fused:
                dz1, parts, n, dw_dw = K.dwconv_bwd_fused(dz2, y2, coef2, w_dw, y1, st1, ACT_SILU, geom.kernel, geom.stride,
                                                          geom.pad_lead, geom.pad_lead, _dest(ctx, 4, (Cmid, 1, kk, kk)))
            else:
                dz1, parts, n = K.dwconv_bwd_data(dz2, y2, coef2, w_dw, y1, st1, ACT_SILU, y1.shape, geom.kernel,
                                                  geom.stride, geom.pad_lead, geom.pad_lead)
            coef1, dg_exp, db_exp = K.bn_bwd_finalize(parts, n, N * H * W, g_exp, st1, tr, need[2] or need[3],
                                                      _dest(ctx, 2, (Cmid,)), _dest(ctx, 3, (Cmid,)))
            pro_dy1 = K.pro_affine2(y1, coef1)
            both = K.pwconv_bwd_fused(dz1, y1, coef1, x, wexp_kn, g if cfg.skip else None, _dest(ctx, 1, (Cmid, Cin))) \
                if (need[0] and need[1] and K.pwconv_bwd_fused_ok(dz1, x)) else None
            with K.side_stream(N * Ho * Wo):
                if need[4] and not fused:
                    dw_dw = K.dwconv_bwd_weight(dz2, y2, coef2, y1, st1, ACT_SILU, geom.kernel, geom.stride,
                                                geom.pad_lead, geom.pad_lead, _dest(ctx, 4, (Cmid, 1, kk, kk)))
                if need[1] and both is None:
                    dw_exp = K.pwconv_wgrad(dz1, pro_dy1, x, None, _dest(ctx, 1, (Cmid, Cin))).view(Cmid, Cin, 1, 1)
            if both is not None:
                dx, dw_exp = both[0], both[1].view(Cmid, Cin, 1, 1)
            elif need[0]:
                dx, _, _ = K.pwconv(dz1, pro_dy1, wexp_kn, g if cfg.skip else None, stats=False)
        else:
            if need[4]:
                with K.side_stream(N * Ho * Wo):
                    dw_dw = K.dwconv_bwd_weight(dz2, y2, coef2, x, None, ACT_NONE, geom.kernel, geom.stride,
                                                geom.pad_lead, geom.pad_lead, _dest(ctx, 4, (Cmid, 1, kk, kk)))
            if need[0]:
                dx, _, _ = K.dwconv_bwd_data(dz2, y2, coef2, w_dw, None, None, ACT_NONE, ctx.in_shape, geom.kernel,
                                             geom.stride, geom.pad_lead, geom.pad_lead)
                if cfg.skip:
                    dx = K.add(dx, g)
        K.join_side()
        return (dx, dw_exp, dg_exp, db_exp, dw_dw, dg_dw, db_dw, dw1, db1, dw2, db2, dw_proj, dg_proj, db_proj,
                None, None)


@dataclass
class HeadCtx:
    bn: BNRef
    dropout: float
    training: bool
    derived: tuple | None = None
    counters: list | None = None


class HeadFunction(torch.autograd.Function):

    @staticmethod
    def forward(ctx, x, w_head, gamma, beta, w_fc, b_fc, drop_u, cfg: HeadCtx):
        N, H, W, Cin = x.shape
        need_bwd = any(ctx.needs_input_grad)
        w_nk, w_kn = cfg.derived if cfg.derived is not None else K.prep_weights(w_head, x.dtype, True, need_bwd)
        y, parts, n = K.pwconv(x, None, w_nk, None, stats=cfg.training)
        st = _bn_state(parts, n, N * H * W, cfg.bn, gamma, beta, cfg.training, cfg.counters)
        pooled = K.pool_act(y, st, ACT_SILU)
        feat = K.dropout(pooled, drop_u, cfg.dropout) if drop_u is not None else pooled
        logits = K.linear_fwd(feat, w_fc, b_fc)
        ctx.cfg = cfg
        ctx.pptr = _ptrs(x, w_head, gamma, beta, w_fc, b_fc)
        ctx.has_bias = b_fc is not None
        ctx.save_for_backward(x, y, st, feat, w_kn, w_fc, gamma, drop_u)
        return logits

    @staticmethod
    def backward(ctx, dlogits):
        cfg: HeadCtx = ctx.cfg
        x, y, st, feat, w_kn, w_fc, gamma, drop_u = ctx.saved_tensors
        need = ctx.needs_input_grad
        N, H, W, Cin = x.shape
        Chead = y.shape[3]
        backbone = need[0] or need[1] or need[2] or need[3]
        J = w_fc.shape[0]
        dfeat, dw_fc, db_fc = K.linear_bwd(_c(dlogits.float()), feat, w_fc, backbone, need[4], ctx.has_bias and need[5],
                                           _dest(ctx, 4, (J, Chead)), _dest(ctx, 5, (J,)) if ctx.has_bias else None)
        dx = dw_head = dgamma = dbeta = None
        if backbone:
            dpooled = K.dropout(dfeat, drop_u, cfg.dropout) if drop_u is not None else dfeat
            dz, parts, n = K.act_bn_bwd(None, y, None, dpooled, st, ACT_SILU)
            coef, dgamma, dbeta = K.bn_bwd_finalize(parts, n, N * H * W, gamma, st, cfg.training, need[2] or need[3],
                                                    _dest(ctx, 2, (Chead,)), _dest(ctx, 3, (Chead,)))
            pro = K.pro_affine2(y, coef)
            if need[0]:
                dx, _, _ = K.pwconv(dz, pro, w_kn, None, stats=False)
            if need[1]:
                dw_head = K.pwconv_wgrad(dz, pro, x, None, _dest(ctx, 1, (Chead, Cin))).view(Chead, Cin, 1, 1)
        return dx, dw_head, dgamma, dbeta, dw_fc, db_fc, None, None

class HeadConvFunction(torch.autograd.Function):

    @staticmethod
    def forward(ctx, x, w_head):
        w_nk, w_kn = K.prep_weights(w_head, x.dtype, True, True)
        y, _, _ = K.pwconv(x, None, w_nk, None, stats=False)
        ctx.save_for_backward(x, w_kn)
        return y

    @staticmethod
    def backward(ctx, g):
        x, w_kn = ctx.saved_tensors
        g = _c(g)
        dx = dw = None
        if ctx.needs_input_grad[0]:
            dx, _, _ = K.pwconv(g, None, w_kn, None, stats=False)
        if ctx.needs_input_grad[1]:
            dw = K.pwconv_wgrad(g, None, x, None).view(g.shape[3], x.shape[3], 1, 1)
        return dx, dw


class HeadTailEvalFunction(torch.autograd.Function):

    @staticmethod
    def forward(ctx, y, w_fc, b_fc, bn: BNRef, gamma, beta):
        st = K.bn_eval_coeffs(bn.params(gamma, beta))
        pooled = K.pool_act(y, st, ACT_SILU)
        logits = K.linear_fwd(pooled, w_fc, b_fc)
        ctx.save_for_backward(y, st, pooled, w_fc)
        return logits

    @staticmethod
    def backward(ctx, dlogits):
        y, st, pooled, w_fc = ctx.saved_tensors
        dy = None
        if ctx.needs_input_grad[0]:
            dpooled, _, _ = K.linear_bwd(_c(dlogits.float()), pooled, w_fc, True, False, False, None, None)
            dz, _, _ = K.act_bn_bwd(None, y, None, dpooled, st, ACT_SILU)
            C = y.shape[3]
            coef = torch.empty((3, C), dtype=torch.float32, device=y.device)
            coef[0].copy_(st[0])
            coef[1:].zero_()
            dy = K.affine2_apply(dz, y, coef)
        return dy, None, None, None, None, None



class CrossEntropyFunction(torch.autograd.Function):

    @staticmethod
    def forward(ctx, logits, targets, label_smoothing: float):
        if targets.is_floating_point():
            if targets.shape != logits.shape:
                raise ValueError(f"probability targets must have the logits' shape {tuple(logits.shape)}, got {tuple(targets.shape)}")
            loss, dlogits = K.ce_loss_soft(_c(logits), _c(targets.float()), label_smoothing, 1.0, ctx.needs_input_grad[0])
# ... 14 lines not shown
```

### deepfakedetection_amd/kernels.py

```python

from __future__ import annotations

import contextlib
import functools
import ctypes
import threading
import weakref
from dataclasses import dataclass

import os

import torch

from . import _lib
from ._lib import (
    ACT_NONE, ACT_SILU, BF16, F32, MAX_PARTIALS, MIX_CUTMIX, MIX_JOB_WORDS, MIX_KEEP, MIX_NCHW, MIX_NHWC, PRO_AFFINE2, PRO_BN_ACT,
    PRO_BN_ACT_GATE, PRO_NONE, DwShape, Prologue, StemShape, check,
)

_scratch: dict[tuple[int, int, str], torch.Tensor] = {}


def _L():
    return _lib.load()
# ... 813 lines not shown
        from ._lib import BnEvalJob

        recs = self._rec
        dev = recs[0][1].running_mean.device
        with torch.inference_mode(False):
            self._flat = torch.empty(sum(4 * k[-1] for k, _ in recs), dtype=torch.float32, device=dev)
        jobs, at, self.states = (BnEvalJob * len(recs))(), 0, []
        for i, (key, _) in enumerate(recs):
            C = key[-1]
            st = self._flat[at:at + 4 * C].view(4, C)
            at += 4 * C
            self.states.append(st)
            jobs[i] = BnEvalJob(key[0], key[1], key[2], key[3], key[4], key[5], st.data_ptr(), key[6], C)
        self._jobs, self.keys = jobs, [k for k, _ in recs]


class EvalBNStates:

    def __init__(self, bns: list) -> None:
        from ._lib import BnEvalJob

        self.ptrs = [(bn.weight.data_ptr(), bn.bias.data_ptr(), bn.running_mean.data_ptr(), bn.running_var.data_ptr()) for bn in bns]
        dev = bns[0].running_mean.device
        total = sum(4 * bn.running_mean.numel() for bn in bns)
        self.flat = torch.empty(total, dtype=torch.float32, device=dev)
        self.states, jobs, at = [], (BnEvalJob * len(bns))(), 0
        for i, bn in enumerate(bns):
            C = bn.running_mean.numel()
            st = self.flat[at:at + 4 * C].view(4, C)
            at += 4 * C
            self.states.append(st)
            jobs[i] = BnEvalJob(bn.weight.data_ptr(), bn.bias.data_ptr(), None, None, bn.running_mean.data_ptr(),
                                bn.running_var.data_ptr(), st.data_ptr(), float(bn.eps), C)
        self._jobs = jobs
        self._tensors = [t for bn in bns for t in (bn.weight, bn.bias, bn.running_mean, bn.running_var)]
        self.fresh = False

    def valid_for(self, bns: list) -> bool:
        return len(bns) == len(self.ptrs) and all(
            (bn.weight.data_ptr(), bn.bias.data_ptr(), bn.running_mean.data_ptr(), bn.running_var.data_ptr()) == p
            for bn, p in zip(bns, self.ptrs))

    def refresh(self) -> None:
        if _journal is not None:
            journal_note(self.flat)
            journal_note(self._tensors)
        check(_L().dfd_bn_eval_coeffs_multi(self._jobs, len(self._jobs), _stream()), "dfd_bn_eval_coeffs_multi")


def pwconv(a: torch.Tensor, pro: Prologue | None, w_nk: torch.Tensor, residual: torch.Tensor | None = None,
           stats: bool = False):
    if isinstance(w_nk, MxWeight):
        if residual is not None or stats:
            raise ValueError("the MX fp8 GEMM has no residual / statistics epilogue")
        aq, asc = mx_quant_rows(a, pro)
        return mx_gemm(aq, asc, w_nk, a.dtype, (*a.shape[:-1], w_nk.N)), None, 0
    K = a.shape[-1]
    M = a.numel() // K
    Nout = w_nk.shape[0]
    out = torch.empty((*a.shape[:-1], Nout), dtype=a.dtype, device=a.device)
    parts = partials_buf(a.device, Nout) if stats else None
    n = ctypes.c_int(0)
    check(_L().dfd_pwconv_fwd(_dt(a), _p(a), ctypes.byref(pro) if pro is not None else None, _p(w_nk), _p(out),
                              _p(residual), M, K, Nout, _p(parts), MAX_PARTIALS, ctypes.byref(n), _stream()),
          "dfd_pwconv_fwd", f"M={M} K={K} N={Nout}")
    return out, parts, n.value


def pwconv_eval(a: torch.Tensor, w_nk: torch.Tensor, out_state: torch.Tensor, out_act: int) -> torch.Tensor:
    K = a.shape[-1]
    M = a.numel() // K
    Nout = w_nk.shape[0]
    out = torch.empty((*a.shape[:-1], Nout), dtype=a.dtype, device=a.device)
    check(_L().dfd_pwconv_fwd_eval(_dt(a), _p(a), _p(w_nk), _p(out_state), out_act, _p(out), M, K, Nout, _stream()),
          "dfd_pwconv_fwd_eval", f"M={M} K={K} N={Nout}")
    return out


def dwconv_eval(x: torch.Tensor, w: torch.Tensor, out_state: torch.Tensor, out_act: int, k: int, stride: int, pad_top: int,
                pad_left: int, Ho: int, Wo: int):
    _chk_nhwc(x)
    N, H, W, C = x.shape
    y = torch.empty((N, Ho, Wo, C), dtype=x.dtype, device=x.device)
    shp = _dw_shape(x.shape, Ho, Wo, k, stride, pad_top, pad_left)
    tiles = _L().dfd_dwconv_fwd_eval_tiles(_dt(x), ctypes.byref(shp))
    if tiles < 1:
        raise ValueError(f"dfd_dwconv_fwd_eval: unsupported shape {tuple(x.shape)} k{k}s{stride}")
    parts = torch.empty((tiles, N, C), dtype=torch.float32, device=x.device)
    n = ctypes.c_int(0)
    check(_L().dfd_dwconv_fwd_eval(_dt(x), _p(x), _p(w), _p(out_state), out_act, _p(y), ctypes.byref(shp), _p(parts),
                                   ctypes.byref(n), _stream()), "dfd_dwconv_fwd_eval", f"{tuple(x.shape)} k{k}s{stride}")
    assert n.value == tiles
    return y, parts, tiles


def se_fwd_parts(parts: torch.Tensor, HW: int, w1, b1, w2, b2, act: int, w2t: torch.Tensor | None = None):
    tiles, N, C = parts.shape
    R = w1.shape[0]
    dev = parts.device
    pooled = torch.empty((N, C), dtype=torch.float32, device=dev)
    hpre = torch.empty((N, R), dtype=torch.float32, device=dev)
    gate = torch.empty((N, C), dtype=torch.float32, device=dev)
    ready = w2t is not None
    if not ready:
        w2t = torch.empty((R, C), dtype=torch.float32, device=dev)
    check(_L().dfd_se_fwd_parts(_p(parts), tiles, N, HW, C, _p(w1), _p(b1), None if ready else _p(w2), _p(b2), R, act,
                                _p(pooled), _p(hpre), _p(gate), _p(w2t), _stream()), "dfd_se_fwd_parts", f"C={C} R={R}")
    return pooled, gate, w2t


def pwconv_wgrad(p: torch.Tensor, pro_p: Prologue | None, q: torch.Tensor, pro_q: Prologue | None,
                 out: torch.Tensor | None = None) -> torch.Tensor:
    Ni, Nj = p.shape[-1], q.shape[-1]
    M = p.numel() // Ni
    nbytes = _L().dfd_pwconv_wgrad_ws(M, Ni, Nj)
    ws = scratch(p.device, "wgrad_ws", nbytes)
    dw = _dst(None if out is None else out.view(Ni, Nj), (Ni, Nj), p.device)
    check(_L().dfd_pwconv_wgrad(_dt(p), _p(p), ctypes.byref(pro_p) if pro_p is not None else None, Ni, _p(q),
                                ctypes.byref(pro_q) if pro_q is not None else None, Nj, M, _p(dw), 0, _p(ws),
                                ws.numel() * 4, _stream()), "dfd_pwconv_wgrad", f"M={M} Ni={Ni} Nj={Nj}")
    return dw


_FUSE_EXPAND_BWD = os.environ.get("DFD_FUSE_EXPAND_BWD", "1") != "0"
_FUSE_EXPAND_WIDE = os.environ.get("DFD_FUSE_EXPAND_WIDE", "0") == "1"


def pwconv_bwd_fused_ok(dz: torch.Tensor, x: torch.Tensor) -> bool:
    Cm, Cin = dz.shape[-1], x.shape[-1]
    M = dz.numel() // Cm
    if not (_FUSE_EXPAND_BWD and dz.dtype == torch.bfloat16 and M >= 2048 * 32 * 3 and Cin <= Cm and Cin % 8 == 0 and Cm % 8 == 0):
        return False
    if Cin <= 32 and (Cm <= 128 or (Cm <= 144 and Cm % 16 == 0)):
        return True
    return _FUSE_EXPAND_WIDE and Cin <= 48 and 144 < Cm <= 240 and Cm % 16 == 0


def pwconv_bwd_fused(dz: torch.Tensor, y: torch.Tensor, coef: torch.Tensor, x: torch.Tensor, w_kn: torch.Tensor,
                     residual: torch.Tensor | None, out_w: torch.Tensor | None = None):
    if not pwconv_bwd_fused_ok(dz, x):
        return None
    Cm, Cin = dz.shape[-1], x.shape[-1]
    M = dz.numel() // Cm
    nbytes = _L().dfd_pwconv_wgrad_ws(M, Cm, Cin)
    ws = scratch(dz.device, "wgrad_ws", nbytes)
    dx = torch.empty_like(x)
    dw = _dst(None if out_w is None else out_w.view(Cm, Cin), (Cm, Cin), dz.device)
    rc = _L().dfd_pwconv_bwd_fused(_dt(dz), _p(dz), _p(y), _p(coef), _p(x), _p(w_kn), _p(residual), M, Cm, Cin, _p(dx), _p(dw), 0,
                                   _p(ws), ws.numel() * 4, _stream())
    check(rc, "dfd_pwconv_bwd_fused", f"M={M} Cm={Cm} Cin={Cin}")
    return dx, dw


def _stem_shape(x_shape, Cout: int, Ho: int, Wo: int, k: int, stride: int, pt: int, pl: int) -> StemShape:
    N, H, W, _ = x_shape
    return StemShape(N, H, W, Cout, Ho, Wo, k, stride, pt, pl)


def stem_conv_fwd(x: torch.Tensor, w: torch.Tensor, out_dtype: torch.dtype, stride: int, pad_top: int, pad_left: int,
                  Ho: int, Wo: int, stats: bool = True):
    _chk_nhwc(x)
    if x.dtype != torch.float32 or x.shape[3] != 3:
        raise ValueError("stem input must be f32 [N,H,W,3]")
    Cout, k = w.shape[0], w.shape[2]
    y = torch.empty((x.shape[0], Ho, Wo, Cout), dtype=out_dtype, device=x.device)
    shp = _stem_shape(x.shape, Cout, Ho, Wo, k, stride, pad_top, pad_left)
    parts = partials_buf(x.device, Cout) if stats else None
    n = ctypes.c_int(0)
    check(_L().dfd_stem_conv_fwd(_dt(y), _p(x), _p(w), _p(y), ctypes.byref(shp), _p(parts), MAX_PARTIALS,
                                 ctypes.byref(n), _stream()), "dfd_stem_conv_fwd")
    return y, parts, n.value


def stem_conv_wgrad(x: torch.Tensor, dz: torch.Tensor, y: torch.Tensor | None, coef: torch.Tensor | None, k: int,
                    stride: int, pad_top: int, pad_left: int, out: torch.Tensor | None = None) -> torch.Tensor:
    Cout, Ho, Wo = dz.shape[3], dz.shape[1], dz.shape[2]
    shp = _stem_shape(x.shape, Cout, Ho, Wo, k, stride, pad_top, pad_left)
    nbytes = _L().dfd_stem_conv_wgrad_ws(ctypes.byref(shp))
    ws = scratch(dz.device, "wgrad_ws", nbytes)
    dw = _dst(out, (Cout, 3, k, k), dz.device)
    check(_L().dfd_stem_conv_wgrad(_dt(dz), _p(x), _p(dz), _p(y), _p(coef), _p(dw), ctypes.byref(shp), 0, _p(ws),
                                   ws.numel() * 4, _stream()), "dfd_stem_conv_wgrad")
    return dw


def dropout(x: torch.Tensor, u: torch.Tensor, p: float) -> torch.Tensor:
    out = torch.empty_like(x)
    check(_L().dfd_dropout(_p(x), _p(u), p, _p(out), x.numel(), _stream()), "dfd_dropout")
    return out


def linear_fwd(x: torch.Tensor, w: torch.Tensor, b: torch.Tensor | None) -> torch.Tensor:
    N, K = x.shape
    J = w.shape[0]
    out = torch.empty((N, J), dtype=torch.float32, device=x.device)
    check(_L().dfd_linear_fwd(_p(x), _p(w), _p(b), _p(out), N, K, J, _stream()), "dfd_linear_fwd")
    return out


def linear_bwd(dout: torch.Tensor, x: torch.Tensor, w: torch.Tensor, need_dx: bool, need_dw: bool, has_bias: bool,
               out_dw: torch.Tensor | None = None, out_db: torch.Tensor | None = None):
    N, K = x.shape
    J = w.shape[0]
    dev = x.device
    dx = torch.empty((N, K), dtype=torch.float32, device=dev) if need_dx else None
    dw = _dst(out_dw, (J, K), dev) if need_dw else None
    db = _dst(out_db, (J,), dev) if (need_dw and has_bias) else None
    check(_L().dfd_linear_bwd(_p(dout), _p(x), _p(w), _p(dx), _p(dw), _p(db), N, K, J, 0, _stream()), "dfd_linear_bwd")
    return dx, dw, db


def ce_loss(logits: torch.Tensor, targets: torch.Tensor, label_smoothing: float, grad_scale: float = 1.0,
            want_grad: bool = True):
    N, J = logits.shape
    dev = logits.device
    row_loss = torch.empty(N, dtype=torch.float32, device=dev)
    loss = torch.empty((), dtype=torch.float32, device=dev)
    dlogits = torch.empty_like(logits) if want_grad else None
    check(_L().dfd_ce_loss(_p(logits), _p(targets), N, J, label_smoothing, grad_scale, _p(row_loss), _p(loss),
                           _p(dlogits), _stream()), "dfd_ce_loss")
    return loss, dlogits


def ce_loss_soft(logits: torch.Tensor, targets: torch.Tensor, label_smoothing: float, grad_scale: float = 1.0,
                 want_grad: bool = True):
    if targets.dtype != torch.float32 or targets.shape != logits.shape:
        raise ValueError(f"ce_loss_soft: targets must be f32 {tuple(logits.shape)}, got {targets.dtype} {tuple(targets.shape)}")
    N, J = logits.shape
    dev = logits.device
    row_loss = torch.empty(N, dtype=torch.float32, device=dev)
    loss = torch.empty((), dtype=torch.float32, device=dev)
    dlogits = torch.empty_like(logits) if want_grad else None
    check(_L().dfd_ce_loss_soft(_p(logits), _p(targets), N, J, label_smoothing, grad_scale, _p(row_loss), _p(loss),
                                _p(dlogits), _stream()), "dfd_ce_loss_soft")
    return loss, dlogits


def softmax_argmax(logits: torch.Tensor, want_probs: bool = True):
    N, J = logits.shape
    probs = torch.empty_like(logits) if want_probs else None
    preds = torch.empty(N, dtype=torch.int64, device=logits.device)
    check(_L().dfd_softmax_argmax(_p(logits), N, J, _p(probs), _p(preds), _stream()), "dfd_softmax_argmax")
    return probs, preds


def gradcam_map(act: torch.Tensor, grad: torch.Tensor) -> torch.Tensor:
    if act.dim() != 4 or act.shape != grad.shape or act.dtype != grad.dtype:
        raise ValueError(f"gradcam_map: act {tuple(act.shape)} {act.dtype} and grad {tuple(grad.shape)} {grad.dtype} must be equal NHWC")
    N, h, w, C = act.shape
    cam = torch.empty((N, h, w), dtype=torch.float32, device=act.device)
    check(_L().dfd_gradcam_map(_p(act), _p(grad), _dt(act), N, h * w, C, _p(cam), _stream()), "dfd_gradcam_map",
          f"{tuple(act.shape)}")
    return cam


def cam_render(cam: torch.Tensor, size: tuple[int, int], image: torch.Tensor | None = None, mean_std: torch.Tensor | None = None,
               lut: torch.Tensor | None = None, image_weight: float = 0.5) -> tuple[torch.Tensor, torch.Tensor | None]:
    N, h, w = cam.shape
    H, W = size
    heat = torch.empty((N, H, W), dtype=torch.float32, device=cam.device)
    overlay = None
    if image is not None:
        if image.dtype != torch.float32 or tuple(image.shape) != (N, 3, H, W):
            raise ValueError(f"cam_render: image must be f32 [{N}, 3, {H}, {W}], got {tuple(image.shape)} {image.dtype}")
        if lut is None or mean_std is None or lut.dtype != torch.uint8 or tuple(lut.shape) != (256, 3) or mean_std.numel() != 6:
            raise ValueError("cam_render: an overlay needs a uint8 [256, 3] lut and f32 [6] mean_std")
        image = image.contiguous()
        overlay = torch.empty((N, H, W, 3), dtype=torch.uint8, device=cam.device)
    ws_bytes = _L().dfd_cam_render_ws(N, h, w, H, W)
    ws = torch.empty(ws_bytes, dtype=torch.uint8, device=cam.device)
    check(_L().dfd_cam_render(_p(cam), N, h, w, H, W, _p(image), _p(mean_std if image is not None else None),
                              _p(lut if image is not None else None), float(image_weight), _p(heat), _p(overlay), _p(ws), ws_bytes,
                              _stream()), "dfd_cam_render", f"{N}x{h}x{w} -> {H}x{W}")
    return heat, overlay


def adamw_step(table: torch.Tensor, hp: torch.Tensor) -> None:
    check(_L().dfd_adamw_step(_p(table), table.shape[0], _p(hp), _stream()), "dfd_adamw_step")


def ema_update(table: torch.Tensor, w: torch.Tensor) -> None:
    check(_L().dfd_ema_update(_p(table), table.shape[0], _p(w), _stream()), "dfd_ema_update")


def check_mix_jobs(jobs: torch.Tensor, N: int, H: int, W: int) -> None:
    if jobs.is_cuda or jobs.dtype != torch.int32 or tuple(jobs.shape) != (N, MIX_JOB_WORDS):
        raise ValueError(f"mix_batch: the job table must be a host int32 [{N}, {MIX_JOB_WORDS}] tensor, got "
                         f"{jobs.dtype} {tuple(jobs.shape)} on {jobs.device}")
    mode, y0, y1, x0, x1 = (jobs[:, c] for c in (0, 3, 4, 5, 6))
    if bool(((mode < MIX_KEEP) | (mode > MIX_CUTMIX)).any()):
        raise ValueError("mix_batch: unknown mode in the job table")
    bad = (y0 < 0) | (y0 > y1) | (y1 > H) | (x0 < 0) | (x0 > x1) | (x1 > W)
    if bool(bad.any()):
        n = int(bad.nonzero()[0])
        raise ValueError(f"mix_batch: job {n}: box rows [{int(y0[n])}, {int(y1[n])}) columns [{int(x0[n])}, {int(x1[n])}) "
                         f"leaves the {H} x {W} picture")
    if N % 2 == 1 and int(mode[N // 2]) != MIX_KEEP:
        raise ValueError("mix_batch: the middle sample of an odd batch is its own partner and must be kept")


def mix_batch(x: torch.Tensor, labels: torch.Tensor, jobs: torch.Tensor, num_classes: int) -> torch.Tensor:
    if not x.is_cuda:
        raise RuntimeError("mix_batch needs the batch on a HIP device (no CPU fallback)")
    if x.dim() != 4 or x.shape[1] != 3 or x.dtype != torch.float32:
        raise ValueError(f"mix_batch: x must be f32 [N, 3, H, W], got {x.dtype} {tuple(x.shape)}")
    N, _, H, W = x.shape
# ... 274 lines not shown
    return out


def conv_weight_to_dgrad_gemm(w: torch.Tensor) -> torch.Tensor:
    O, I, k, _ = w.shape
    out = torch.empty((I, k * k * O), dtype=torch.float32, device=w.device)
    check(_L().dfd_conv_weight_perm(_p(w), _p(out), O, I, k, 2, 0, _stream()), "dfd_conv_weight_perm")
    return out


def conv_wgrad_from_gemm(dw_gemm: torch.Tensor, shape, out: torch.Tensor | None = None) -> torch.Tensor:
    O, I, k, _ = shape
    dw = _dst(out, (O, I, k, k), dw_gemm.device)
    check(_L().dfd_conv_weight_perm(_p(dw_gemm), _p(dw), O, I, k, 0, 0, _stream()), "dfd_conv_weight_perm")
    return dw


def layernorm_fwd(x: torch.Tensor, gamma: torch.Tensor, beta: torch.Tensor, eps: float, want_stats: bool = True):
    rows, C = _rows_c(x)
    y = torch.empty_like(x)
    stats = torch.empty((rows, 2), dtype=torch.float32, device=x.device) if want_stats else None
    check(_L().dfd_layernorm_fwd(_dt(x), _p(x), _p(gamma), _p(beta), eps, _p(y), _p(stats), rows, C, _stream()), "dfd_layernorm_fwd")
    return y, stats


def layernorm_bwd(g: torch.Tensor, x: torch.Tensor, gamma: torch.Tensor, stats: torch.Tensor, residual: torch.Tensor | None = None,
                  out2: torch.Tensor | None = None):
    rows, C = _rows_c(x)
    dx = torch.empty_like(x)
    parts = partials_buf(x.device, C)
    n = ctypes.c_int(0)
    check(_L().dfd_layernorm_bwd(_dt(x), _p(g), _p(x), _p(gamma), _p(stats), _p(residual), _p(dx), _p(parts), MAX_PARTIALS,
                                 ctypes.byref(n), rows, C, _stream()), "dfd_layernorm_bwd")
    if out2 is not None:
        if tuple(out2.shape) != (2, C) or out2.dtype != torch.float32 or not out2.is_contiguous():
            raise ValueError("layernorm_bwd: out2 must be a contiguous f32 [2, C] tensor")
        check(_L().dfd_sum_rows_deferred(_p(parts), n.value, 2 * C, _p(out2), 0, _stream()), "dfd_sum_rows_deferred")
        return dx, out2[0], out2[1]
    both = torch.empty((2, C), dtype=torch.float32, device=x.device)
    sum_rows(parts, n.value, 2 * C, both)
    return dx, both[0], both[1]


def copy_rows(src: torch.Tensor, sidx: torch.Tensor | None, dst: torch.Tensor, didx: torch.Tensor | None, n: int) -> torch.Tensor:
    C = src.shape[-1]
    if dst.shape[-1] != C or src.dtype != dst.dtype:
        raise ValueError("copy_rows: source and destination rows differ")
    check(_L().dfd_copy_rows(_dt(src), _p(src), _p(sidx), _p(dst), _p(didx), n, C, _stream()), "dfd_copy_rows")
    return dst


def add_rowtable(x: torch.Tensor, table: torch.Tensor) -> torch.Tensor:
    T, C = table.shape
    out = torch.empty_like(x)
    check(_L().dfd_add_rowtable(_dt(x), _p(x), _p(table), _p(out), x.numel() // C, T, C, _stream()), "dfd_add_rowtable")
    return out


def rowtable_grad(g: torch.Tensor, T: int) -> torch.Tensor:
    C = g.shape[-1]
    dtable = torch.empty((T, C), dtype=torch.float32, device=g.device)
    nbytes = int(_L().dfd_rowtable_grad_ws(T, C))
    ws = scratch(g.device, "rowtable_ws", nbytes)
    check(_L().dfd_rowtable_grad(_dt(g), _p(g), _p(dtable), g.numel() // C, T, C, 0, _p(ws), nbytes, _stream()),
          "dfd_rowtable_grad")
    return dtable


def avgpool_fwd(x: torch.Tensor, k: int, stride: int) -> torch.Tensor:
    _chk_nhwc(x)
    N, H, W, C = x.shape
    out = torch.empty((N, (H - k) // stride + 1, (W - k) // stride + 1, C), dtype=x.dtype, device=x.device)
    check(_L().dfd_avgpool_fwd(_dt(x), _p(x), _p(out), N, H, W, k, stride, C, _stream()), "dfd_avgpool_fwd")
    return out


def avgpool_bwd(g: torch.Tensor, in_shape, k: int, stride: int) -> torch.Tensor:
    N, H, W, C = in_shape
    dx = torch.empty((N, H, W, C), dtype=g.dtype, device=g.device)
    check(_L().dfd_avgpool_bwd(_dt(g), _p(g), _p(dx), N, H, W, k, stride, C, _stream()), "dfd_avgpool_bwd")
    return dx


def relpos_bias_fwd(table: torch.Tensor, idx: torch.Tensor, n_local: int, n_global: int) -> torch.Tensor:
    H = table.shape[1]
    S = n_local + n_global
    full = torch.empty((H, S, S), dtype=torch.float32, device=table.device)
    check(_L().dfd_relpos_bias_fwd(_p(table), _p(idx), _p(full), H, n_local, n_global, _stream()), "dfd_relpos_bias_fwd")
    return full


def relpos_bias_bwd(dfull: torch.Tensor, table: torch.Tensor, idx: torch.Tensor, n_local: int, n_global: int) -> torch.Tensor:
    T, H = table.shape
    dtable = torch.empty_like(table)
    check(_L().dfd_relpos_bias_bwd(_p(dfull), _p(table), _p(idx), _p(dtable), H, T, n_local, n_global, _stream()), "dfd_relpos_bias_bwd")
    return dtable


def axpby(x: torch.Tensor, y: torch.Tensor | None, a: float = 1.0, b: float = 1.0, a_dev: torch.Tensor | None = None,
          out: torch.Tensor | None = None) -> torch.Tensor:
    out = torch.empty_like(x) if out is None else out
    check(_L().dfd_axpby(_p(x), _p(y), a, b, _p(a_dev), _p(out), x.numel(), _stream()), "dfd_axpby")
    return out


def add(a: torch.Tensor, b: torch.Tensor) -> torch.Tensor:
    out = torch.empty_like(a)
    check(_L().dfd_add(_dt(a), _p(a), _p(b), _p(out), a.numel(), _stream()), "dfd_add")
    return out


class DeviceRng:

    def __init__(self, device: torch.device, seed: int | None = None) -> None:
        with torch.inference_mode(False):
            self.state = torch.zeros(2, dtype=torch.int64, device=device)
        self.reseed(seed)
        self._counter_key: tuple = ()
        self._counter_table: torch.Tensor | None = None

    @staticmethod
    def mix_seed(seed: int, rank: int) -> int:
        return (seed ^ (rank * 0x9E3779B97F4A7C15)) & 0x7FFFFFFFFFFFFFFF

    def reseed(self, seed: int | None = None, rank: int | None = None) -> None:
        seed = torch.initial_seed() if seed is None else seed
        rank = int(os.environ.get("RANK", "0")) if rank is None else rank
        host = torch.tensor([self.mix_seed(seed, rank), 0], dtype=torch.int64)
        with torch.inference_mode(False):
            self.state.copy_(host)

    def uniform(self, n: int, stream_id: int) -> torch.Tensor:
        out = torch.empty(n, dtype=torch.float32, device=self.state.device)
        check(_L().dfd_rand(_p(self.state), stream_id, 0.0, _p(out), n, _stream()), "dfd_rand")
        return out

    def drop_path_scale(self, n: int, keep: float, stream_id: int) -> torch.Tensor:
        out = torch.empty(n, dtype=torch.float32, device=self.state.device)
        check(_L().dfd_rand(_p(self.state), stream_id, keep, _p(out), n, _stream()), "dfd_rand")
        return out

    def tick(self, counters: list[torch.Tensor]) -> None:
        key = tuple(c.data_ptr() for c in counters)
        if key != self._counter_key:
            self._counter_key = key
            with torch.inference_mode(False):
                self._counter_table = torch.tensor(list(key), dtype=torch.int64).to(self.state.device) if key else None
        journal_note(counters)
        check(_L().dfd_step_tick(_p(self._counter_table), len(key), _p(self.state), _stream()), "dfd_step_tick")


_profile_sink: list | None = None
_TIMED = ("bn_act_apply", "bn_bwd_reduce", "act_bn_bwd", "pool_act", "pool_bwd_reduce", "scale_rows", "dwconv_fwd",
          "dwconv_bwd_data", "dwconv_bwd_weight", "dwconv_bwd_fused", "pwconv", "pwconv_wgrad", "pwconv_bwd_fused", "stem_conv_fwd", "stem_conv_wgrad",
          "se_fc_fwd", "se_fc_bwd", "linear_fwd", "linear_bwd", "ce_loss", "adamw_step", "prep_weights", "bn_finalize",
          "bn_bwd_finalize", "bn_bwd_finalize_ex", "dropout", "bgemm", "attn_scores", "attn_apply", "attn_softmax_fwd", "attn_softmax_bwd", "im2col", "col2im",
          "wattn_fwd", "wattn_bwd", "mx_quant_rows", "mx_gemm",
          "bn_add_act", "bn_add_act_bwd", "affine2_apply", "up2_act_fwd", "up2_act_bwd", "layernorm_fwd", "layernorm_bwd",
          "channel_stats", "subsample_add")


def set_profile_sink(sink: list | None) -> None:
    global _profile_sink
    _profile_sink = sink


def _tensor_bytes(obj) -> int:
    if isinstance(obj, torch.Tensor):
        if obj.dim() <= 1 and obj.numel() >= MAX_PARTIALS:
            return 0
        return obj.numel() * obj.element_size()
    if isinstance(obj, Prologue):
        return getattr(obj, "_nbytes", 0)
    if isinstance(obj, (tuple, list)):
        return sum(_tensor_bytes(o) for o in obj)
    return 0


def _flops(name: str, args) -> float:
    if name == "pwconv":
        a, w = args[0], args[2]
        return 2.0 * (a.numel() // a.shape[-1]) * a.shape[-1] * w.shape[0]
    if name == "pwconv_wgrad":
        p, q = args[0], args[2]
        return 2.0 * (p.numel() // p.shape[-1]) * p.shape[-1] * q.shape[-1]
    if name == "pwconv_bwd_fused":
        dz, x = args[0], args[3]
        return 4.0 * (dz.numel() // dz.shape[-1]) * dz.shape[-1] * x.shape[-1]
    return 0.0


def _bytes_8d(name: str, args, fallback: int) -> int:
    try:
        if name == "pwconv":
            a, w = args[0], args[2]
            K_, es = a.shape[-1], a.element_size()
            M = a.numel() // K_
            return (M * K_ + M * w.shape[0]) * es + w.numel() * es
        if name == "pwconv_wgrad":
            p, q = args[0], args[2]
            M = p.numel() // p.shape[-1]
            return M * (p.shape[-1] + q.shape[-1]) * p.element_size() + p.shape[-1] * q.shape[-1] * 4
        if name == "pwconv_bwd_fused":
            dz, x = args[0], args[3]
            Cm, Cin, es = dz.shape[-1], x.shape[-1], dz.element_size()
            M = dz.numel() // Cm
            return 2 * M * (Cm + Cin) * es + Cm * Cin * (es + 4)
        if name == "dwconv_fwd":
            x, k, Ho, Wo = args[0], args[4], args[8], args[9]
            N, H, W, C = x.shape
            return N * C * (H * W + Ho * Wo) * x.element_size() + k * k * C * 4
        if name == "dwconv_bwd_data":
            dz, xin, in_shape = args[0], args[4], args[7]
            N, H, W, C = in_shape
            return N * C * (dz.shape[1] * dz.shape[2] + H * W * (2 if xin is not None else 1)) * dz.element_size()
        if name == "dwconv_bwd_weight":
            dz, xin = args[0], args[3]
            N, H, W, C = xin.shape
            return N * C * (dz.shape[1] * dz.shape[2] + H * W) * dz.element_size()
    except (IndexError, AttributeError, TypeError):
        pass
    return fallback


def _timed(name: str, fn):
    def inner(*args, **kwargs):
        sink = _profile_sink
        if sink is None:
            return fn(*args, **kwargs)
        e0, e1 = torch.cuda.Event(enable_timing=True), torch.cuda.Event(enable_timing=True)
        e0.record()
        out = fn(*args, **kwargs)
        e1.record()
        nbytes = _tensor_bytes(args) + _tensor_bytes(list(kwargs.values())) + _tensor_bytes(out)
        sink.append((name, nbytes, _flops(name, args), e0, e1, _bytes_8d(name, args, nbytes)))
        return out

    inner.__name__ = name
    inner.__doc__ = fn.__doc__
    return inner


for _name in _TIMED:
    globals()[_name] = _timed(_name, globals()[_name])

__all__ = [name for name in dir() if not name.startswith("_")]
```

### include/dfd_hip.h

```cpp
#ifndef DFD_HIP_H
#define DFD_HIP_H

#include <stddef.h>
#include <stdint.h>

#ifdef __cplusplus
extern "C" {
#endif

typedef void* dfd_stream;

#define DFD_OK            0
#define DFD_EINVAL       (-1)
#define DFD_EUNSUPPORTED (-2)
#define DFD_ELAUNCH      (-3)
#define DFD_EWORKSPACE   (-4)

#define DFD_F32   0
#define DFD_BF16  1

#define DFD_ACT_NONE 0
#define DFD_ACT_SILU 1
#define DFD_ACT_RELU 2
#define DFD_ACT_GELU 3

#define DFD_MAX_PARTIALS 1024

#define DFD_BNSTATE_ROWS 4
#define DFD_BNCOEF_ROWS  3

int dfd_version(void);

int dfd_tune(int key, int value);

int dfd_sum_batch_begin(void);
int dfd_sum_batch_end(void);
int dfd_sum_batch_end_deferred(void);
int dfd_sum_passengers_flush(dfd_stream stream);
int dfd_sum_passengers_discard(void);


int dfd_bn_finalize(const float* partials, int nparts, int C, double count,
                    const float* gamma, const float* beta,
                    float* running_mean, float* running_var, float momentum, float eps,
                    float* bnstate, dfd_stream stream);
int dfd_bn_eval_coeffs(const float* gamma, const float* beta, const float* running_mean,
                       const float* running_var, float eps, int C, float* bnstate,
                       dfd_stream stream);
typedef struct {
    const float *gamma, *beta, *conv_bias, *ls, *running_mean, *running_var;
    float* bnstate;
    float eps;
    int C;
} dfd_bn_eval_job;
int dfd_bn_eval_coeffs_multi(const dfd_bn_eval_job* jobs, int njobs, dfd_stream stream);
int dfd_bn_bwd_finalize(const float* partials, int nparts, int C, double count,
                        const float* gamma, const float* bnstate, int train,
                        float* dgamma, float* dbeta, int accumulate, float* coef,
                        dfd_stream stream);

int dfd_bn_finalize_ex(const float* partials, int nparts, int C, double count, const float* gamma,
                       const float* beta, const float* conv_bias, const float* ls_gamma,
                       float* running_mean, float* running_var, float momentum, float eps,
                       float* bnstate, dfd_stream stream);
int dfd_bn_eval_coeffs_ex(const float* gamma, const float* beta, const float* conv_bias,
                          const float* ls_gamma, const float* running_mean, const float* running_var,
                          float eps, int C, float* bnstate, dfd_stream stream);
int dfd_bn_bwd_finalize_ex(const float* partials, int nparts, int C, double count, const float* gamma,
                           const float* beta, const float* ls_gamma, const float* bnstate, int train,
                           float* dgamma, float* dbeta, float* dls, float* dbias, int accumulate,
                           float* coef, dfd_stream stream);

int dfd_bn_act_apply(int dtype, const void* y, const float* bnstate, int act,
                     const void* residual, const float* row_scale, void* out,
                     int N, int HW, int C, dfd_stream stream);
int dfd_bn_bwd_reduce(int dtype, const void* g, const void* y, const float* bnstate,
                      const float* row_scale, int N, int HW, int C,
                      float* partials, int pcap, int* nparts, dfd_stream stream);
int dfd_gemm_bias_act(int dtype, const void* a, const void* w_nk, int M, int K, int N, const float* state, int act,
                      const void* residual, const float* row_scale, int HW, void* yraw, void* out, dfd_stream stream);
int dfd_gemm_plan(int M, int K, int N);
int dfd_pw_ntd_plan(int M, int K, int Nout);
size_t dfd_bias_grad_ws(int N, int HW, int C);
int dfd_bias_grad(int dtype, const void* g, const float* row_scale, int N, int HW, int C, float* dbias, int accumulate,
                  float* ws, size_t ws_bytes, dfd_stream stream);
int dfd_act_bn_bwd(int dtype, const void* D, const void* y, const float* gate,
                   const float* dpool, const float* bnstate, int act, void* dz,
                   int N, int HW, int C, float* partials, int pcap, int* nparts,
                   dfd_stream stream);
int dfd_act_bn_bwd_se(int dtype, const void* D, const void* y, const float* gate, const float* dpool,
                      const float* bnstate, int act, void* dz, int N, int HW, int C, float* partials, int pcap,
                      int* nparts, const float* se_pooled, const float* se_ws, int R, float* dw1, float* db1, float* dw2,
                      float* db2, int accumulate, dfd_stream stream);
size_t dfd_pool_ws(int dtype, int N, int HW, int C);
int dfd_pool_act(int dtype, const void* y, const float* bnstate, int act, float* pooled,
                 int N, int HW, int C, void* ws, size_t ws_bytes, dfd_stream stream);
int dfd_pool_bwd_reduce(int dtype, const void* D, const void* y, const float* bnstate,
                        int act, float* dgate, int N, int HW, int C, void* ws, size_t ws_bytes,
                        dfd_stream stream);
int dfd_scale_rows(int dtype, const void* x, const float* row_scale, void* out,
                   int N, int HW, int C, dfd_stream stream);

int dfd_se_fc_fwd(const float* pooled, const float* w1, const float* b1, const float* w2,
                  const float* b2, int N, int C, int R, int act, float* hpre, float* gate,
                  float* w2t, dfd_stream stream);
int dfd_se_fc_bwd(const float* dgate, const float* gate, const float* hpre,
                  const float* pooled, const float* w1, const float* w2t,
                  int N, int C, int R, int act, float* dpooled,
                  float* dw1, float* db1, float* dw2, float* db2, int accumulate,
                  float* ws, dfd_stream stream);
int dfd_se_fwd(int dtype, const void* y, const float* bnstate, int act_in, int N, int HW, int C,
               const float* w1, const float* b1, const float* w2, const float* b2, int R, int act,
               float* pooled, float* hpre, float* gate, float* w2t, void* ws, size_t ws_bytes,
               dfd_stream stream);
int dfd_se_bwd(int dtype, const void* D, const void* y, const float* bnstate, int act_in, int N, int HW,
               int C, const float* gate, const float* hpre, const float* pooled, const float* w1,
               const float* w2t, int R, int act, float* dgate, float* dpooled, float* dw1, float* db1,
               float* dw2, float* db2, int accumulate, void* pool_ws, size_t pool_ws_bytes, float* ws,
               dfd_stream stream);

typedef struct {
    int N, H, W, C;
    int Ho, Wo;
    int k, stride, pad_top, pad_left;
} dfd_dwconv_shape;

int dfd_dwconv_fwd(int dtype, const void* x, const float* in_bnstate, int in_act,
                   const float* w, void* y, const dfd_dwconv_shape* s,
                   float* partials, int pcap, int* nparts, dfd_stream stream);
int dfd_dwconv_bwd_data(int dtype, const void* dz, const void* y, const float* coef,
                        const float* w, const void* xin, const float* in_bnstate, int in_act,
                        void* dzin, const dfd_dwconv_shape* s,
                        float* partials, int pcap, int* nparts, dfd_stream stream);
int dfd_dwconv_bwd_weight(int dtype, const void* dz, const void* y, const float* coef,
                          const void* xin, const float* in_bnstate, int in_act,
                          float* dw, const dfd_dwconv_shape* s, int accumulate,
                          float* ws, size_t ws_bytes, dfd_stream stream);

int dfd_dw_mm_plan(const dfd_dwconv_shape* s, int pro, int* out);

int dfd_pwconv_fwd_eval(int dtype, const void* a, const void* w, const float* out_bnstate, int out_act,
                        void* out, int M, int K, int Nout, dfd_stream stream);
int dfd_dwconv_fwd_eval_tiles(int dtype, const dfd_dwconv_shape* s);
int dfd_dwconv_fwd_eval(int dtype, const void* x, const float* w, const float* out_bnstate, int out_act, void* y,
                        const dfd_dwconv_shape* s, float* pool_parts, int* ntiles, dfd_stream stream);
int dfd_se_fwd_parts(const float* parts, int splits, int N, int HW, int C, const float* w1, const float* b1,
                     const float* w2, const float* b2, int R, int act, float* pooled, float* hpre, float* gate,
                     float* w2t, dfd_stream stream);
size_t dfd_dwconv_bwd_weight_ws(const dfd_dwconv_shape* s);
int dfd_dwconv_bwd_fused(int dtype, const void* dz, const void* y, const float* coef, const float* w, const void* xin,
                         const float* in_bnstate, int in_act, void* dzin, float* dw, const dfd_dwconv_shape* s,
                         float* partials, int pcap, int* nparts, int accumulate, float* ws, size_t ws_bytes,
                         dfd_stream stream);

#define DFD_PRO_NONE        0
#define DFD_PRO_BN_ACT      1
#define DFD_PRO_BN_ACT_GATE 2
#define DFD_PRO_AFFINE2     3
typedef struct {
    int mode;
    int act;
    int HW;
    int _pad;
    const void* a2;
    const float* coef;
    const float* gate;
} dfd_prologue;

int dfd_pwconv_fwd(int dtype, const void* a, const dfd_prologue* pro, const void* w,
                   void* out, const void* residual, int M, int K, int Nout,
                   float* partials, int pcap, int* nparts, dfd_stream stream);
int dfd_pwconv_wgrad(int dtype, const void* p, const dfd_prologue* pro_p, int Ni,
                     const void* q, const dfd_prologue* pro_q, int Nj, int M,
                     float* dw, int accumulate, float* ws, size_t ws_bytes,
                     dfd_stream stream);
int dfd_pwconv_bwd_fused(int dtype, const void* dz, const void* y, const float* coef, const void* x, const void* w_kn,
                         const void* residual, int M, int Cm, int Cin, void* dx, float* dw, int accumulate, float* ws,
                         size_t ws_bytes, dfd_stream stream);
size_t dfd_pwconv_wgrad_ws(int M, int Ni, int Nj);
int dfd_pw_prep_weights(int dtype, const float* w, void* w_nk, void* w_kn, int N, int K,
                        dfd_stream stream);
typedef struct dfd_prep_job {
    const float* src;
    void* nk;
    void* kn;
    int N, K;
    int dtype;
    int _pad;
} dfd_prep_job;
int dfd_prep_weights_multi(const dfd_prep_job* jobs, int njobs, dfd_stream stream);

typedef struct {
    int N, H, W, Cout, Ho, Wo, k, stride, pad_top, pad_left;
} dfd_stem_shape;
int dfd_stem_conv_fwd(int dtype, const float* x, const float* w, void* y,
                      const dfd_stem_shape* s, float* partials, int pcap, int* nparts,
                      dfd_stream stream);
int dfd_stem_conv_wgrad(int dtype, const float* x, const void* dz, const void* y,
                        const float* coef, float* dw, const dfd_stem_shape* s,
                        int accumulate, float* ws, size_t ws_bytes, dfd_stream stream);
size_t dfd_stem_conv_wgrad_ws(const dfd_stem_shape* s);

int dfd_dropout(const float* x, const float* u, float p, float* out, int n, dfd_stream stream);
int dfd_linear_fwd(const float* x, const float* w, const float* b, float* out,
                   int N, int K, int J, dfd_stream stream);
int dfd_linear_bwd(const float* dout, const float* x, const float* w, float* dx,
                   float* dw, float* db, int N, int K, int J, int accumulate,
                   dfd_stream stream);
int dfd_ce_loss(const float* logits, const int64_t* targets, int N, int J,
                float label_smoothing, float grad_scale, float* row_loss, float* loss,
                float* dlogits, dfd_stream stream);
int dfd_ce_loss_soft(const float* logits, const float* targets, int N, int J,
                     float label_smoothing, float grad_scale, float* row_loss, float* loss,
                     float* dlogits, dfd_stream stream);
int dfd_softmax_argmax(const float* logits, int N, int J, float* probs, int64_t* preds,
                       dfd_stream stream);
typedef struct dfd_resize_job {
    long offset;
    int H, W;
    int bx, by, bw, bh;
    int rw, rh;
    int cx, cy;
    int _pad[2];
} dfd_resize_job;
int dfd_resize_crop_u8(const unsigned char* src, const dfd_resize_job* jobs_dev, unsigned char* dst, int N, int OH, int OW,
                       int max_shrink, dfd_stream stream);
typedef struct {
    int mode;
    int a[6];
    int order[4];
    float fb, fc, fs;
    int dh;
    int enable;
} dfd_augment_job;
int dfd_augment_u8(const unsigned char* src, const dfd_augment_job* jobs_dev, unsigned char* dst, int N, int H, int W,
                   dfd_stream stream);
#define DFD_AUG_MAX_OPS 4
#define DFD_AUG_IDENTITY     0
#define DFD_AUG_SHEAR_X      1
#define DFD_AUG_SHEAR_Y      2
#define DFD_AUG_TRANSLATE_X  3
#define DFD_AUG_TRANSLATE_Y  4
#define DFD_AUG_ROTATE       5
#define DFD_AUG_BRIGHTNESS   6
#define DFD_AUG_COLOR        7
#define DFD_AUG_CONTRAST     8
#define DFD_AUG_SHARPNESS    9
#define DFD_AUG_POSTERIZE    10
#define DFD_AUG_SOLARIZE     11
#define DFD_AUG_AUTOCONTRAST 12
#define DFD_AUG_EQUALIZE     13
#define DFD_AUG_NUM_OPS      14
typedef struct {
    int op;
    int ip;
    float fp;
    int a[6];
} dfd_augment_op;
typedef struct {
    dfd_augment_job base;
    int flip;
    int nops;
    dfd_augment_op ops[DFD_AUG_MAX_OPS];
} dfd_augment_policy_job;
int dfd_augment_policy_u8(const unsigned char* src, const dfd_augment_policy_job* jobs_host, const dfd_augment_policy_job* jobs_dev,
                          unsigned char* dst, int N, int H, int W, dfd_stream stream);

int dfd_image_prep(const unsigned char* src, float* dst, int N, int H, int W, const float* mean3,
                   const float* std3, const unsigned char* flip, const int* erase, dfd_stream stream);
#define DFD_ADAMW_TABLE_COLS 5
#define DFD_ADAMW_HP_LEN 8
int dfd_adamw_step(const int64_t* table, int nchunks, const float* hp, dfd_stream stream);
#define DFD_EMA_TABLE_COLS 4
#define DFD_EMA_LERP 0
#define DFD_EMA_COPY 1
int dfd_ema_update(const int64_t* table, int nchunks, const float* w, dfd_stream stream);
#define DFD_MIX_JOB_WORDS 8
#define DFD_MIX_KEEP 0
#define DFD_MIX_MIXUP 1
#define DFD_MIX_CUTMIX 2
#define DFD_MIX_NHWC 0
#define DFD_MIX_NCHW 1
int dfd_mix_batch(float* x, const int64_t* labels, const int32_t* jobs, float* y, int N, int H, int W, int J, int layout,
                  dfd_stream stream);


int dfd_affine2_apply(int dtype, const void* dz, const void* y, const float* coef, void* out, long rows,
                      int C, dfd_stream stream);
int dfd_bn_add_act(int dtype, const void* y, const float* bnstate, const void* other, int act, void* out,
                   long rows, int C, dfd_stream stream);
int dfd_bn_add_act_bwd(int dtype, const void* g, const void* y, const float* bnstate, const void* other,
                       int act, void* d, long rows, int C, float* partials, int pcap, int* nparts,
                       dfd_stream stream);
int dfd_channel_stats(int dtype, const void* x, long rows, int C, float* partials, int pcap, int* nparts,
                      dfd_stream stream);
int dfd_sum_rows(float* partials, int P, long L, float* out, int accumulate, dfd_stream stream);
int dfd_sum_rows_deferred(float* partials, int P, long L, float* out, int accumulate, dfd_stream stream);
int dfd_up2_act_fwd(int dtype, const void* s, int act, void* out, int N, int h, int w, int C, dfd_stream stream);
int dfd_up2_act_bwd(int dtype, const void* g, const void* s, int act, void* ds, int N, int h, int w, int C,
                    void* ws, dfd_stream stream);
int dfd_subsample_add(int dtype, const void* a, const float* bias, const void* x, void* out, int N, int H,
                      int W, int stride, int C, dfd_stream stream);
int dfd_subsample_add_bwd(int dtype, const void* g, void* dx, int N, int H, int W, int stride, int C,
                          dfd_stream stream);

typedef struct { long sb, sh, sr, sc; } dfd_mat;
int dfd_bgemm(int dt_a, const void* A, const dfd_mat* sa, int dt_b, const void* B, const dfd_mat* sb,
              int dt_c, void* C, const dfd_mat* sc, const float* bias, float alpha, int nb, int nh, int M,
              int N, int K, int round_a, int round_b, dfd_stream stream);
int dfd_attn_softmax_fwd(const float* S, const float* th_w1, const float* th_b1, const float* th_w2,
                         const float* th_b2, float* P, float* T2, int B, int H, int Nq, int Nk,
                         dfd_stream stream);
int dfd_attn_softmax_bwd(const float* dT2, const float* P, const float* th_w1, const float* th_w2,
                         float* dT1, float* dS, int B, int H, int Nq, int Nk, dfd_stream stream);
int dfd_bias_gather(const float* table, const int* idx, float* full, int H, int T, long L, dfd_stream stream);
int dfd_bias_scatter(const float* dfull, const int* idx, float* dtable, int H, int T, long L, int accumulate,
                     dfd_stream stream);

int dfd_conv_fwd(int dtype, const void* x, const dfd_dwconv_shape* s, const float* in_bnstate, int in_act,
                 const void* w_nk, int Cout, void* y, float* partials, int pcap, int* nparts, dfd_stream stream);

size_t dfd_conv_wgrad_ws(const dfd_dwconv_shape* s, int Cout);
int dfd_conv_wgrad(int dtype, const void* p, const dfd_prologue* pro_p, int Cout, const void* x,
                   const dfd_dwconv_shape* s, const float* in_bnstate, int in_act, float* dw, int accumulate,
                   float* ws, size_t ws_bytes, dfd_stream stream);

int dfd_im2col(int dtype, const void* x, const float* in_bnstate, int in_act, void* col,
               const dfd_dwconv_shape* s, dfd_stream stream);
int dfd_col2im(int dtype, const void* dcol, void* dx, const dfd_dwconv_shape* s, dfd_stream stream);
int dfd_conv_weight_perm(const float* src, float* dst, int O, int I, int k, int to_gemm, int accumulate,
                         dfd_stream stream);
// ... 86 lines not shown
```

Before: 20440 images/sec.

## Fuse projection-conv backward with data grad, weight grad and SE pool reduction

Adds a fused projection pointwise-conv backward kernel for the Cmid=32 block (the first MBConv stage). In one pass it computes the weight gradient, the data gradient D via MFMA against staged weights, and per-wave partial sums of D times the activation for the SE backward pool. The SE backward then consumes these partials directly. This replaces the separate affine2_apply, pwconv, side-stream wgrad and pool-reduction passes over the large early-stage activation tensors. The cost is a more complex kernel with tight shape preconditions (image-aligned row partitions), and an env flag can disable it.

```diff
diff --git a/deepfakedetection_amd/_lib.py b/deepfakedetection_amd/_lib.py
--- a/deepfakedetection_amd/_lib.py
+++ b/deepfakedetection_amd/_lib.py
@@ -101,6 +101,10 @@
     "dfd_mix_batch": (c_int, [P, P, P, P, c_int, c_int, c_int, c_int, c_int, P]),
     "dfd_ce_loss_soft": (c_int, [P, P, c_int, c_int, c_float, c_float, P, P, P, P]),
     "dfd_augment_policy_u8": (c_int, [P, P, P, P, c_int, c_int, c_int, P]),
+    "dfd_pwconv_proj_bwd_plan": (c_int, [c_int, c_int, c_int, c_int, c_int, P, P]),
+    "dfd_pwconv_proj_bwd_fused": (c_int, [c_int, P, P, P, P, P, c_int, P, P, c_int, c_int, c_int, c_int, P, P, c_int, P, c_size_t,
+                                          P, c_size_t, P, P]),
+    "dfd_se_bwd_parts": (c_int, [P, c_int, c_int, c_int, P, P, P, P, P, c_int, c_int, P, P, P, P, P, c_int, P, P]),
     "dfd_bn_eval_coeffs_multi": (c_int, [P, c_int, P]),
     "dfd_sum_batch_begin": (c_int, []),
     "dfd_sum_batch_end": (c_int, []),
diff --git a/deepfakedetection_amd/csrc/dfd_misc.hip b/deepfakedetection_amd/csrc/dfd_misc.hip
--- a/deepfakedetection_amd/csrc/dfd_misc.hip
+++ b/deepfakedetection_amd/csrc/dfd_misc.hip
@@ -304,6 +304,25 @@
     DISPATCH_ACT(act, {
         hipLaunchKernelGGL((k_se_bwd_img<ACT>), dim3(N), dim3(SE_IMG_THREADS), 0, st, (const float*)pool_ws, splits, dgate, gate, hpre,
                            w1, w2t, N, C, R, ws, dpooled);
+    });
+    if (hipGetLastError() != hipSuccess) return DFD_ELAUNCH;
+    if (dw1 && dw2) {
+        hipLaunchKernelGGL(k_se_fc_bwd_w, dim3((C + 63) / 64, R), dim3(DFD_THREADS), 0, st, pooled, ws, N, C, R, dw1, db1,
+                           dw2, db2, accumulate);
+    }
+    return DFD_CHECK_LAUNCH();
+}
+
+extern "C" int dfd_se_bwd_parts(const float* parts, int splits, int N, int C, const float* gate, const float* hpre, const float* pooled,
+                                const float* w1, const float* w2t, int R, int act, float* dpooled, float* dw1, float* db1, float* dw2,
+                                float* db2, int accumulate, float* ws, dfd_stream stream) {
+    if (!parts || splits < 1 || !gate || !hpre || !pooled || !w1 || !w2t || !dpooled || !ws || N < 1 || C < 1 || R < 1 || C % 4)
+        return DFD_EINVAL;
+    if (C > SE_MAX_C || R > SE_MAX_R) return DFD_EUNSUPPORTED;
+    hipStream_t st = (hipStream_t)stream;
+    DISPATCH_ACT(act, {
+        hipLaunchKernelGGL((k_se_bwd_img<ACT>), dim3(N), dim3(SE_IMG_THREADS), 0, st, parts, splits, parts, gate, hpre, w1, w2t, N, C, R,
+                           ws, dpooled);
     });
     if (hipGetLastError() != hipSuccess) return DFD_ELAUNCH;
     if (dw1 && dw2) {
diff --git a/deepfakedetection_amd/csrc/dfd_pwtnw.hip b/deepfakedetection_amd/csrc/dfd_pwtnw.hip
--- a/deepfakedetection_amd/csrc/dfd_pwtnw.hip
+++ b/deepfakedetection_amd/csrc/dfd_pwtnw.hip
@@ -6,7 +6,11 @@
 __global__ void __launch_bounds__(DFD_THREADS, NBT > 9 ? 1 : 2)
 k_pw_tnw(const bf16* __restrict__ a, ProArgs pa, int Na, const bf16* __restrict__ b, ProArgs pb, int Nb, int M,
          int rows_per_block, int swap, float* __restrict__ ws, const bf16* __restrict__ w_kn = nullptr,
-         const bf16* __restrict__ res = nullptr, bf16* __restrict__ dx = nullptr, int wstride = 0, int woff = 0) {
+         const bf16* __restrict__ res = nullptr, bf16* __restrict__ dx = nullptr, int wstride = 0, int woff = 0,
+         float* __restrict__ pool_parts = nullptr, int nsp = 1, int nwaves = 0) {
+    constexpr bool XG = DG == 1 || DG == 2;
+    constexpr bool PJ = DG >= 3, POOL = DG == 4;
+    static_assert(!PJ || (ROWS == 32 && NBT == 2 && NA == 2), "projection backward: Cmid = 32, Cout <= 32");
     constexpr int ITA = (ROWS * NA * 2 + 63) / 64;
     constexpr int ITB = (ROWS * NBT * 2 + 63) / 64;
     extern __shared__ __attribute__((aligned(16))) unsigned char smem[];
@@ -17,6 +21,9 @@
     const bf16* a2 = reinterpret_cast<const bf16*>(pa.a2);
     const bf16* b2 = reinterpret_cast<const bf16*>(pb.a2);
     const int ca = Na >> 3, cb = Nb >> 3;
+    unsigned char* atile = PJ ? bt : at;
+    const int aoff = PJ ? cb : 0;
+    auto a0_at = [&](int row, int ch) -> unsigned char* { return at + tn_off_bf16(row, ch); };
     float* gc = cl + 3 * (Na + Nb) + wave * 2 * Nb;
     int gimg = -1;
 
@@ -28,7 +35,16 @@
         cl[3 * Na + i] = v;
     }
     for (int i = t; i < 4 * 2 * ROWS * 256 / 16; i += DFD_THREADS) reinterpret_cast<uint4*>(smem)[i] = make_uint4(0, 0, 0, 0);
-    if constexpr (DG) {
+    if constexpr (PJ) {
+        const int chunks = wstride >> 4;
+        for (int i = t; i < NBT * 16 * chunks; i += DFD_THREADS) {
+            const int r = i / chunks, c = i - r * chunks;
+            uint4 v = make_uint4(0, 0, 0, 0);
+            if (r < Nb && c < ca) v = *reinterpret_cast<const uint4*>(w_kn + (long)r * Na + c * 8);
+            *reinterpret_cast<uint4*>(smem + woff + r * wstride + c * 16) = v;
+        }
+    }
+    if constexpr (XG) {
         const int chunks = wstride >> 4;
         for (int i = t; i < NA * 16 * chunks; i += DFD_THREADS) {
             const int r = i / chunks, c = i - r * chunks;
@@ -62,7 +78,15 @@
         for (int y = 0; y < NBT; ++y) acc[x][y] = (f32x4_t){0.f, 0.f, 0.f, 0.f};
     const int na = (Na + 15) >> 4, nbt = (Nb + 15) >> 4;
     constexpr int RT = ROWS / 16;
-    f32x4_t accd[DG ? NA : 1][RT];
+    f32x4_t accd[XG ? NA : 1][RT];
+    const int erg = lane >> 2, ecg = lane & 3;
+    float psum[POOL ? 4 : 1][8];
+    if constexpr (POOL) {
+#pragma unroll
+        for (int k = 0; k < 4; ++k)
+#pragma unroll
+            for (int j = 0; j < 8; ++j) psum[k][j] = 0.f;
+    }
 
     const int rows_per_wave = rows_per_block / 4;
     const int mbeg = blockIdx.x * rows_per_block + wave * rows_per_wave;
@@ -90,7 +114,7 @@
 #pragma unroll
         for (int i = 0; i < ITB; ++i) load_b(i, m0);
     };
-    auto pro_item = [&](auto mode_tag, uint4 q, uint4 q2, const float* cf, int N, int ch, int m, const ProArgs& pr) -> uint4 {
+    auto pro_item = [&](auto mode_tag, uint4 q, uint4 q2, const float* cf, int N, int ch, int m, const ProArgs& pr, uint4& a0q) -> uint4 {
         constexpr int MODE = decltype(mode_tag)::value;
         if constexpr (MODE == DFD_PRO_NONE) {
             return q;
@@ -111,8 +135,16 @@
                 float gt[8];
                 load_f32<8>(gc + (pro_image(pr, m) - gimg) * N + ch * 8, gt);
                 bn_act_array<ACT, 8>(v, c0, c1);
-#pragma unroll
-                for (int j = 0; j < 8; ++j) v[j] = round_to<bf16>(v[j]) * gt[j];
+                if constexpr (POOL) {
+#pragma unroll
+                    for (int j = 0; j < 8; ++j) v[j] = round_to<bf16>(v[j]);
+                    a0q = f_to_q(v);
+#pragma unroll
+                    for (int j = 0; j < 8; ++j) v[j] *= gt[j];
+                } else {
+#pragma unroll
+                    for (int j = 0; j < 8; ++j) v[j] = round_to<bf16>(v[j]) * gt[j];
+                }
             }
             return f_to_q(v);
         }
@@ -121,9 +153,9 @@
 #pragma unroll
         for (int i = 0; i < ITA; ++i) {
             if (ra[i] >= 0) {
-                uint4 v = make_uint4(0, 0, 0, 0);
-                if (m0 + ra[i] < mend) v = pro_item(std::integral_constant<int, PA>{}, va[i], va2[i], cl, Na, cha[i], m0 + ra[i], pa);
-                *reinterpret_cast<uint4*>(at + tn_off_bf16(ra[i], cha[i])) = v;
+                uint4 v = make_uint4(0, 0, 0, 0), unused;
+                if (m0 + ra[i] < mend) v = pro_item(std::integral_constant<int, PA>{}, va[i], va2[i], cl, Na, cha[i], m0 + ra[i], pa, unused);
+                *reinterpret_cast<uint4*>(atile + tn_off_bf16(ra[i], aoff + cha[i])) = v;
             }
             load_a(i, m0 + ROWS);
         }
@@ -133,10 +165,12 @@
 #pragma unroll
         for (int i = 0; i < ITB; ++i) {
             if (rb[i] >= 0 && (chb[i] >> 4) == grp) {
-                uint4 v = make_uint4(0, 0, 0, 0);
-                if (m0 + rb[i] < mend)
-                    v = pro_item(std::integral_constant<int, PB>{}, vb[i], vb2[i], cl + 3 * Na, Nb, chb[i], m0 + rb[i], pb);
-                *reinterpret_cast<uint4*>(bt + tn_off_bf16(rb[i], chb[i] & 15)) = v;
+                const int r_ = rb[i], c_ = chb[i];
+                uint4 v = make_uint4(0, 0, 0, 0), a0q = make_uint4(0, 0, 0, 0);
+                if (m0 + r_ < mend)
+                    v = pro_item(std::integral_constant<int, PB>{}, vb[i], vb2[i], cl + 3 * Na, Nb, c_, m0 + r_, pb, a0q);
+                *reinterpret_cast<uint4*>(bt + tn_off_bf16(r_, c_ & 15)) = v;
+                if constexpr (POOL) *reinterpret_cast<uint4*>(a0_at(r_, c_)) = a0q;
             }
             if constexpr (refill) load_b(i, m0 + ROWS);
         }
@@ -186,7 +220,7 @@
                 wave_sync();
             }
         }
-        if constexpr (DG) {
+        if constexpr (XG) {
 #pragma unroll
             for (int x = 0; x < NA; ++x)
 #pragma unroll
@@ -197,7 +231,15 @@
         wave_sync();
 #pragma unroll
         for (int x = 0; x < NA; ++x)
-            if (x < na) fa[x] = frag(at, 2 * x);
+            if (x < na) fa[x] = frag(atile, aoff + 2 * x);
+        uint4 fd3[PJ ? RT : 1];
+        if constexpr (PJ) {
+#pragma unroll
+            for (int j = 0; j < RT; ++j) {
+                fd3[j] = *reinterpret_cast<const uint4*>(atile + tn_off_bf16(j * 16 + li, aoff + g));
+                if (g >= ca) fd3[j] = make_uint4(0, 0, 0, 0);
+            }
+        }
 #pragma unroll
         for (int grp = 0; grp < NGRP; ++grp) {
             if (grp > 0) {
@@ -214,7 +256,49 @@
                     if (x < na)
                         acc[x][y] = mma(fa[x], fb, acc[x][y]);
             }
-            if constexpr (DG) {
+            if constexpr (PJ) {
+                wave_sync();
+#pragma unroll
+                for (int y = 0; y < NBT; ++y) {
+                    if ((y >> 3) != grp || y >= nbt) continue;
+                    const uint4 fw = *reinterpret_cast<const uint4*>(smem + woff + (y * 16 + li) * wstride + g * 16);
+                    const int pch = 2 * (y & 7) + (g >> 1);
+                    const bool pok = 2 * y + (g >> 1) < cb;
+#pragma unroll
+                    for (int j = 0; j < RT; ++j) {
+                        const f32x4_t d = __builtin_amdgcn_mfma_f32_16x16x32_bf16(__builtin_bit_cast(bf16x8_t, fw), __builtin_bit_cast(bf16x8_t, fd3[j]),
+                                                                                  (f32x4_t){0.f, 0.f, 0.f, 0.f}, 0, 0, 0);
+                        if (pok)
+                            *reinterpret_cast<uint2*>(bt + tn_off_bf16(j * 16 + li, pch) + ((g & 1) << 3)) =
+                                make_uint2(pack_bf2(d[0], d[1]), pack_bf2(d[2], d[3]));
+                    }
+                }
+                wave_sync();
+#pragma unroll
+                for (int u = 0; u < 2; ++u) {
+                    const int r = erg + 16 * u, m = m0 + r;
+                    if (m < mend) {
+                        const uint4 dq = *reinterpret_cast<const uint4*>(bt + tn_off_bf16(r, ecg));
+                        *reinterpret_cast<uint4*>(dx + (long)m * Nb + ecg * 8) = dq;
+                        if constexpr (POOL) {
+                            float dv[8], av[8];
+                            q_to_f(dq, dv);
+                            q_to_f(*reinterpret_cast<const uint4*>(a0_at(r, ecg)), av);
+#pragma unroll
+                            for (int j = 0; j < 8; ++j) psum[u][j] += av[j] * dv[j];
+                        }
+                    }
+                }
+                if constexpr (POOL) {
+#pragma unroll
+                    for (int j = 0; j < 8; ++j) {
+                        const float t0 = psum[0][j], t1 = psum[1][j];
+                        psum[0][j] = psum[2][j]; psum[1][j] = psum[3][j];
+                        psum[2][j] = t0; psum[3][j] = t1;
+                    }
+                }
+            }
+            if constexpr (XG) {
 #pragma unroll
                 for (int ks = 0; ks < 4; ++ks) {
                     if (grp * 8 + 2 * ks >= NBT || grp * 8 + 2 * ks >= nbt) continue;
@@ -237,7 +321,7 @@
                 }
             }
         }
-        if constexpr (DG) {
+        if constexpr (XG) {
 #pragma unroll
             for (int j = 0; j < RT; ++j) {
                 const int m = m0 + j * 16 + li;
@@ -261,6 +345,26 @@
         wave_sync();
     }
 
+    if constexpr (POOL) {
+        float* pr = reinterpret_cast<float*>(at);
+        const int w = blockIdx.x * 4 + wave;
+        const int img = w / nsp, part = w - img * nsp, nimg = nwaves / nsp;
+        const int odd = mbeg < mend ? ((mend - mbeg + ROWS - 1) / ROWS) & 1 : 0;
+        wave_sync();
+#pragma unroll
+        for (int k = 0; k < 4; ++k) {
+            const int cls = erg + 16 * ((k + 2 * odd) & 3);
+#pragma unroll
+            for (int j = 0; j < 8; ++j) pr[cls * 32 + ecg * 8 + j] = psum[k][j];
+        }
+        wave_sync();
+        if (lane < 32 && w < nwaves) {
+            float sum = 0.f;
+            for (int c = 0; c < 64; ++c) sum += pr[c * 32 + lane];
+            pool_parts[((long)part * nimg + img) * Nb + lane] = sum;
+        }
+    }
+
     __syncthreads();
     float* red = reinterpret_cast<float*>(smem);
     for (int w = 0; w < 4; ++w) {
@@ -296,16 +400,21 @@
             mode_wide == DFD_PRO_BN_ACT);
 }
 
+static void tnw_partition(long M, int rows, int* nblocks, int* rpb) {
+    long r = (M + 511) / 512;
+    r = (r + 4 * rows - 1) / (4 * rows) * (4 * rows);
+    *rpb = (int)r;
+    *nblocks = (int)((M + r - 1) / r);
+}
+
 template <int ROWS, int NA, int NBT>
 static int tnw_launch(const void* a, const dfd_prologue* pro_a, int Na, const void* b, const dfd_prologue* pro_b, int Nb,
                       int M, int swap, float* dw, int accumulate, float* ws, size_t ws_bytes, hipStream_t st) {
     const ProArgs pa = pro_args(pro_a), pb = pro_args(pro_b);
     const int ma = pro_a ? pro_a->mode : DFD_PRO_NONE, mb = pro_b ? pro_b->mode : DFD_PRO_NONE;
     const int act = ((mb == DFD_PRO_BN_ACT_GATE || mb == DFD_PRO_BN_ACT) && pro_b) ? pro_b->act : DFD_ACT_NONE;
-    int nblocks = 512;
-    int rpb = (M + nblocks - 1) / nblocks;
-    rpb = (rpb + 4 * ROWS - 1) / (4 * ROWS) * (4 * ROWS);
-    nblocks = (M + rpb - 1) / rpb;
+    int nblocks, rpb;
+    tnw_partition(M, ROWS, &nblocks, &rpb);
     if ((size_t)(nblocks + nblocks / 32 + 2) * Na * Nb * 4 > ws_bytes) return DFD_EUNSUPPORTED;
     const bool gated = mb == DFD_PRO_BN_ACT_GATE;
     if (gated && pb.HW < ROWS) return DFD_EUNSUPPORTED;
@@ -377,6 +486,65 @@
     return tnw_dg_launch<16, 3, 15>(x, Cin, dz, &pro, Cm, w_kn, residual, M, dx, dw, accumulate, ws, ws_bytes, st);
 }
 
+static int pj_parts(int dtype, int N, int HW, int Cout, int Cmid) {
+    if (dtype != DFD_BF16 || N < 1 || HW < 1 || Cout < 8 || Cout % 8 || Cout > 32 || Cmid != 32) return 0;
+    const long M = (long)N * HW;
+    if (M < 2048 * 32 * 3 || M >= (1l << 31)) return 0;
+    const size_t pb = dfd_pool_ws(DFD_BF16, N, HW, Cmid);
+    const int s = pb ? (int)(pb / ((size_t)N * Cmid * 4)) : 1;
+    if (s < 2 || HW % s) return 0;
+    const int rp = HW / s;
+    if (rp % 32 || rp < 96 || (N * s) % 4) return 0;
+    int nblocks, rpb;
+    tnw_partition(M, 32, &nblocks, &rpb);
+    return rpb == 4 * rp ? s : 0;
+}
+extern "C" int dfd_pwconv_proj_bwd_plan(int dtype, int N, int HW, int Cout, int Cmid, int* parts, size_t* pool_parts_bytes) {
+    const int s = pj_parts(dtype, N, HW, Cout, Cmid);
+    if (!s) return DFD_EUNSUPPORTED;
+    if (parts) *parts = s;
+    if (pool_parts_bytes) *pool_parts_bytes = (size_t)s * N * Cmid * 4;
+    return DFD_OK;
+}
+
+template <int DGV>
+static int tnw_pj_launch(const void* g, const dfd_prologue* pro_g, int Cout, const void* y2, const dfd_prologue* pro_y, int Cmid,
+                         const void* w_kn, int N, int HW, int parts, void* D, float* dw, int accumulate, float* ws, size_t ws_bytes,
+                         float* pool_parts, hipStream_t st) {
+    const ProArgs pa = pro_args(pro_g), pb = pro_args(pro_y);
+    const int M = N * HW, nwaves = N * parts, rpw = HW / parts;
+    const int nblocks = nwaves / 4;
+    if ((size_t)(nblocks + nblocks / 32 + 2) * Cout * Cmid * 4 > ws_bytes) return DFD_EUNSUPPORTED;
+    const int wstride = 80;
+    int woff = 4 * 2 * 32 * 256 + 3 * (Cout + Cmid) * 4 + 4 * 2 * Cmid * 4;
+    woff = (woff + 15) / 16 * 16;
+    const int lds = woff + 2 * 16 * wstride;
+    auto kern = k_pw_tnw<32, 2, 2, DFD_PRO_AFFINE2, DFD_PRO_BN_ACT_GATE, DFD_ACT_SILU, DGV>;
+    struct TnwPjTag;
+    dfd_allow_lds_once<TnwPjTag>(kern, 80 * 1024);
+    hipLaunchKernelGGL(kern, dim3(nblocks), dim3(DFD_THREADS), lds, st, (const bf16*)g, pa, Cout, (const bf16*)y2, pb, Cmid, M, 4 * rpw, 0,
+                       ws, (const bf16*)w_kn, (const bf16*)nullptr, (bf16*)D, wstride, woff, pool_parts, parts, nwaves);
+    if (hipGetLastError() != hipSuccess) return DFD_ELAUNCH;
+    return dfd_launch_sum_partials(ws, nblocks, (long)Cout * Cmid, dw, accumulate, st);
+}
+extern "C" int dfd_pwconv_proj_bwd_fused(int dtype, const void* g, const void* y3, const float* coef3, const void* y2,
+                                         const float* bnstate2, int act, const float* gate, const void* w_kn, int N, int HW, int Cout,
+                                         int Cmid, void* D, float* dw, int accumulate, float* ws, size_t ws_bytes, float* pool_parts,
+                                         size_t pool_parts_bytes, int* parts, dfd_stream stream) {
+    if (!g || !y3 || !coef3 || !y2 || !bnstate2 || !gate || !w_kn || !D || !dw || !ws || N < 1 || HW < 1 || Cout < 1 || Cmid < 1)
+        return DFD_EINVAL;
+    const int s = act == DFD_ACT_SILU ? pj_parts(dtype, N, HW, Cout, Cmid) : 0;
+    if (!s) return DFD_EUNSUPPORTED;
+    if (pool_parts && pool_parts_bytes < (size_t)s * N * Cmid * 4) return DFD_EINVAL;
+    dfd_prologue pg{}, py{};
+    pg.mode = DFD_PRO_AFFINE2; pg.act = DFD_ACT_NONE; pg.HW = 1; pg.a2 = y3; pg.coef = coef3; pg.gate = nullptr;
+    py.mode = DFD_PRO_BN_ACT_GATE; py.act = DFD_ACT_SILU; py.HW = HW; py.a2 = nullptr; py.coef = bnstate2; py.gate = gate;
+    hipStream_t st = (hipStream_t)stream;
+    if (parts) *parts = s;
+    return pool_parts ? tnw_pj_launch<4>(g, &pg, Cout, y2, &py, Cmid, w_kn, N, HW, s, D, dw, accumulate, ws, ws_bytes, pool_parts, st)
+                      : tnw_pj_launch<3>(g, &pg, Cout, y2, &py, Cmid, w_kn, N, HW, s, D, dw, accumulate, ws, ws_bytes, nullptr, st);
+}
+
 int dfd_pw_tnw(const void* p, const dfd_prologue* pro_p, int Ni, const void* q, const dfd_prologue* pro_q, int Nj, int M,
                float* dw, int accumulate, float* ws, size_t ws_bytes, hipStream_t st) {
     if (M < 2048 * 32 * 3) return DFD_EUNSUPPORTED;
diff --git a/deepfakedetection_amd/csrc/dfd_rowpass.hip b/deepfakedetection_amd/csrc/dfd_rowpass.hip
--- a/deepfakedetection_amd/csrc/dfd_rowpass.hip
+++ b/deepfakedetection_amd/csrc/dfd_rowpass.hip
@@ -705,4 +705,4 @@
                                   nullptr, accumulate, coef, stream);
 }
 
-extern "C" int dfd_version(void) { return 139; }
+extern "C" int dfd_version(void) { return 140; }
diff --git a/deepfakedetection_amd/functions.py b/deepfakedetection_amd/functions.py
--- a/deepfakedetection_amd/functions.py
+++ b/deepfakedetection_amd/functions.py
@@ -233,16 +233,24 @@
         Cout, R = y3.shape[3], w1.shape[0]
         coef3, dg_proj, db_proj = K.bn_bwd_finalize(parts, n, N * Ho * Wo, g_proj, st3, tr, need[12] or need[13],
                                                     _dest(ctx, 12, (Cout,)), _dest(ctx, 13, (Cout,)))
-        gm3 = K.affine2_apply(gb, y3, coef3)
-        D, _, _ = K.pwconv(gm3, None, wproj_kn, None, stats=False)
-        dw_proj = None
-        if need[11]:
-            pro_q = K.pro_bn_act_gate(st2, ACT_SILU, gate, Ho * Wo)
-            with K.side_stream(N * Ho * Wo):
-                dw_proj = K.pwconv_wgrad(gm3, None, y2, pro_q, _dest(ctx, 11, (Cout, Cmid))).view(Cout, Cmid, 1, 1)
         want_se = need[7] or need[8] or need[9] or need[10]
         se_outs = (_dest(ctx, 7, (R, Cmid)), _dest(ctx, 8, (R,)), _dest(ctx, 9, (Cmid, R)), _dest(ctx, 10, (Cmid,)))
-        se_res = K.se_bwd(D, y2, st2, ACT_SILU, gate, hpre, pooled, w1, w2t, ACT_SILU, want_se, se_outs, defer_wgrad=SE_WGRAD_PASSENGER)
+        proj = K.pwconv_proj_bwd_fused(gb, y3, coef3, y2, st2, gate, wproj_kn, _dest(ctx, 11, (Cout, Cmid))) \
+            if (need[11] and K.pwconv_proj_bwd_plan(y2.dtype, N, Ho * Wo, Cout, Cmid) is not None) else None
+        if proj is not None:
+            D, dw_proj, pool_parts, nparts = proj
+            dw_proj = dw_proj.view(Cout, Cmid, 1, 1)
+            se_res = K.se_bwd_parts(pool_parts, nparts, gate, hpre, pooled, w1, w2t, ACT_SILU, want_se, se_outs,
+                                    defer_wgrad=SE_WGRAD_PASSENGER)
+        else:
+            gm3 = K.affine2_apply(gb, y3, coef3)
+            D, _, _ = K.pwconv(gm3, None, wproj_kn, None, stats=False)
+            dw_proj = None
+            if need[11]:
+                pro_q = K.pro_bn_act_gate(st2, ACT_SILU, gate, Ho * Wo)
+                with K.side_stream(N * Ho * Wo):
+                    dw_proj = K.pwconv_wgrad(gm3, None, y2, pro_q, _dest(ctx, 11, (Cout, Cmid))).view(Cout, Cmid, 1, 1)
+            se_res = K.se_bwd(D, y2, st2, ACT_SILU, gate, hpre, pooled, w1, w2t, ACT_SILU, want_se, se_outs, defer_wgrad=SE_WGRAD_PASSENGER)
         dpooled, dw1, db1, dw2, db2 = se_res[:5]
         se_job = se_res[5] if SE_WGRAD_PASSENGER else None
         dz2, parts, n = K.act_bn_bwd(D, y2, gate, dpooled, st2, ACT_SILU, se_job=se_job)
diff --git a/deepfakedetection_amd/kernels.py b/deepfakedetection_amd/kernels.py
--- a/deepfakedetection_amd/kernels.py
+++ b/deepfakedetection_amd/kernels.py
@@ -989,6 +989,65 @@
     return dx, dw
 
 
+_FUSE_PROJ_BWD = os.environ.get("DFD_FUSE_PROJ_BWD", "1") != "0"
+_proj_plans: dict = {}
+
+
+def pwconv_proj_bwd_plan(dtype: torch.dtype, N: int, HW: int, Cout: int, Cmid: int):
+    if not _FUSE_PROJ_BWD or dtype != torch.bfloat16:
+        return None
+    key = (N, HW, Cout, Cmid)
+    if key not in _proj_plans:
+        parts, nbytes = ctypes.c_int(0), ctypes.c_size_t(0)
+        rc = _L().dfd_pwconv_proj_bwd_plan(BF16, N, HW, Cout, Cmid, ctypes.byref(parts), ctypes.byref(nbytes))
+        _proj_plans[key] = (parts.value, nbytes.value) if rc == 0 else None
+    return _proj_plans[key]
+
+
+def pwconv_proj_bwd_fused(g: torch.Tensor, y3: torch.Tensor, coef3: torch.Tensor, y2: torch.Tensor, state2: torch.Tensor,
+                          gate: torch.Tensor, w_kn: torch.Tensor, out_w: torch.Tensor | None = None, want_pool: bool = True):
+    _chk_nhwc(y2)
+    N, H, W, Cmid = y2.shape
+    Cout = g.shape[-1]
+    plan = pwconv_proj_bwd_plan(y2.dtype, N, H * W, Cout, Cmid)
+    if plan is None:
+        return None
+    dev = y2.device
+    ws = scratch(dev, "wgrad_ws", _L().dfd_pwconv_wgrad_ws(N * H * W, Cout, Cmid))
+    pool = scratch(dev, "proj_pool_parts", plan[1]) if want_pool else None
+    D = torch.empty_like(y2)
+    dw = _dst(None if out_w is None else out_w.view(Cout, Cmid), (Cout, Cmid), dev)
+    parts = ctypes.c_int(0)
+    rc = _L().dfd_pwconv_proj_bwd_fused(_dt(y2), _p(g), _p(y3), _p(coef3), _p(y2), _p(state2), ACT_SILU, _p(gate), _p(w_kn), N, H * W,
+                                        Cout, Cmid, _p(D), _p(dw), 0, _p(ws), ws.numel() * 4, _p(pool), plan[1] if want_pool else 0,
+                                        ctypes.byref(parts), _stream())
+    check(rc, "dfd_pwconv_proj_bwd_fused", f"N={N} HW={H * W} Cout={Cout} Cmid={Cmid}")
+    return D, dw, pool, parts.value
+
+
+def se_bwd_parts(parts: torch.Tensor, splits: int, gate, hpre, pooled, w1, w2t, act: int, want_param_grads: bool = True,
+                 outs=(None, None, None, None), defer_wgrad: bool = False):
+    N, C = pooled.shape
+    R = w1.shape[0]
+    dev = pooled.device
+    dpooled = torch.empty((N, C), dtype=torch.float32, device=dev)
+    ws = scratch(dev, "se_ws", (N * C + 2 * N * R) * 4)
+    if want_param_grads:
+        dw1 = _dst(outs[0], (R, C), dev)
+        db1 = _dst(outs[1], (R,), dev)
+        dw2 = _dst(outs[2], (C, R), dev)
+        db2 = _dst(outs[3], (C,), dev)
+    else:
+        dw1 = db1 = dw2 = db2 = None
+    defer = defer_wgrad and want_param_grads
+    check(_L().dfd_se_bwd_parts(_p(parts), splits, N, C, _p(gate), _p(hpre), _p(pooled), _p(w1), _p(w2t), R, act, _p(dpooled),
+                                None if defer else _p(dw1), None if defer else _p(db1), None if defer else _p(dw2),
+                                None if defer else _p(db2), 0, _p(ws), _stream()), "dfd_se_bwd_parts")
+    if defer_wgrad:
+        return dpooled, dw1, db1, dw2, db2, ((pooled, ws, R, dw1, db1, dw2, db2) if defer else None)
+    return dpooled, dw1, db1, dw2, db2
+
+
 def _stem_shape(x_shape, Cout: int, Ho: int, Wo: int, k: int, stride: int, pt: int, pl: int) -> StemShape:
     N, H, W, _ = x_shape
     return StemShape(N, H, W, Cout, Ho, Wo, k, stride, pt, pl)
@@ -1569,8 +1628,8 @@
 
 _profile_sink: list | None = None
 _TIMED = ("bn_act_apply", "bn_bwd_reduce", "act_bn_bwd", "pool_act", "pool_bwd_reduce", "scale_rows", "dwconv_fwd",
-          "dwconv_bwd_data", "dwconv_bwd_weight", "dwconv_bwd_fused", "pwconv", "pwconv_wgrad", "pwconv_bwd_fused", "stem_conv_fwd", "stem_conv_wgrad",
-          "se_fc_fwd", "se_fc_bwd", "linear_fwd", "linear_bwd", "ce_loss", "adamw_step", "prep_weights", "bn_finalize",
+          "dwconv_bwd_data", "dwconv_bwd_weight", "dwconv_bwd_fused", "pwconv", "pwconv_wgrad", "pwconv_bwd_fused", "pwconv_proj_bwd_fused",
+          "stem_conv_fwd", "stem_conv_wgrad", "se_fc_fwd", "se_fc_bwd", "linear_fwd", "linear_bwd", "ce_loss", "adamw_step", "prep_weights", "bn_finalize",
           "bn_bwd_finalize", "bn_bwd_finalize_ex", "dropout", "bgemm", "attn_scores", "attn_apply", "attn_softmax_fwd", "attn_softmax_bwd", "im2col", "col2im",
           "wattn_fwd", "wattn_bwd", "mx_quant_rows", "mx_gemm",
           "bn_add_act", "bn_add_act_bwd", "affine2_apply", "up2_act_fwd", "up2_act_bwd", "layernorm_fwd", "layernorm_bwd",
@@ -1604,6 +1663,9 @@
     if name == "pwconv_bwd_fused":
         dz, x = args[0], args[3]
         return 4.0 * (dz.numel() // dz.shape[-1]) * dz.shape[-1] * x.shape[-1]
+    if name == "pwconv_proj_bwd_fused":
+        g, y2 = args[0], args[3]
+        return 4.0 * (y2.numel() // y2.shape[-1]) * y2.shape[-1] * g.shape[-1]
     return 0.0
 
 
@@ -1623,6 +1685,11 @@
             Cm, Cin, es = dz.shape[-1], x.shape[-1], dz.element_size()
             M = dz.numel() // Cm
             return 2 * M * (Cm + Cin) * es + Cm * Cin * (es + 4)
+        if name == "pwconv_proj_bwd_fused":
+            g, y2 = args[0], args[3]
+            Cout, Cm, es = g.shape[-1], y2.shape[-1], y2.element_size()
+            M = y2.numel() // Cm
+            return M * (3 * Cout + 2 * (Cout + Cm) + 2 * Cm) * es + Cm * Cout * (es + 4)
         if name == "dwconv_fwd":
             x, k, Ho, Wo = args[0], args[4], args[8], args[9]
             N, H, W, C = x.shape
diff --git a/include/dfd_hip.h b/include/dfd_hip.h
--- a/include/dfd_hip.h
+++ b/include/dfd_hip.h
@@ -118,6 +118,9 @@
                const float* w2t, int R, int act, float* dgate, float* dpooled, float* dw1, float* db1,
                float* dw2, float* db2, int accumulate, void* pool_ws, size_t pool_ws_bytes, float* ws,
                dfd_stream stream);
+int dfd_se_bwd_parts(const float* parts, int splits, int N, int C, const float* gate, const float* hpre,
+                     const float* pooled, const float* w1, const float* w2t, int R, int act, float* dpooled,
+                     float* dw1, float* db1, float* dw2, float* db2, int accumulate, float* ws, dfd_stream stream);
 
 typedef struct {
     int N, H, W, C;
@@ -177,6 +180,11 @@
 int dfd_pwconv_bwd_fused(int dtype, const void* dz, const void* y, const float* coef, const void* x, const void* w_kn,
                          const void* residual, int M, int Cm, int Cin, void* dx, float* dw, int accumulate, float* ws,
                          size_t ws_bytes, dfd_stream stream);
+int dfd_pwconv_proj_bwd_plan(int dtype, int N, int HW, int Cout, int Cmid, int* parts, size_t* pool_parts_bytes);
+int dfd_pwconv_proj_bwd_fused(int dtype, const void* g, const void* y3, const float* coef3, const void* y2,
+                              const float* bnstate2, int act, const float* gate, const void* w_kn, int N, int HW, int Cout,
+                              int Cmid, void* D, float* dw, int accumulate, float* ws, size_t ws_bytes, float* pool_parts,
+                              size_t pool_parts_bytes, int* parts, dfd_stream stream);
 size_t dfd_pwconv_wgrad_ws(int M, int Ni, int Nj);
 int dfd_pw_prep_weights(int dtype, const float* w, void* w_nk, void* w_kn, int N, int K,
                         dfd_stream stream);
```

Result: faster. 20700 images/sec, median of 6 (+1.2%).
